# cristianpjensen/thesis-pai-reconstruction

Measured on NVIDIA B200. Metric: pix2pix_gan_train_images_per_sec_256x256, higher is better.
Workload: dtype bf16

## Files before the change

include/pai_b200.h:

```cpp
#ifndef PAI_B200_H
#define PAI_B200_H

#ifdef __cplusplus
extern "C" {
#endif

#define PAI_ACT_NONE 0
#define PAI_ACT_LEAKY 1
#define PAI_ACT_RELU 2
#define PAI_ACT_TANH 3

#define PAI_DTYPE_F32 0
#define PAI_DTYPE_BF16 1

const char* pai_last_error(void);
int pai_version(void);
int pai_reserve_sms(int n);

int pai_conv4x4_fprop(const void* x, int n, int h, int w, int cin, int x_ld, const void* w_packed, int cout,
                      int cout_pad, int stride, const float* bias, int act, float slope, void* y, int y_ld,
                      int y_f32, int n_tile, float* splitk_ws, void* stream);

int pai_conv4x4_fprop_dual(const void* x, int n, int h, int w, int cin, int x_ld, const void* w_packed, int cout,
                           int cout_pad, int stride, const float* bias, int act, float slope, void* y, int y_ld, void* y2,
                           int y2_ld, int act2, int n_tile, void* stream);

int pai_convT4x4s2_fprop(const void* x, int n, int h, int w, int cin, int x_ld, const void* w_packed, int cout,
                         int cout_pad, const float* bias, int act, float slope, void* y, int y_ld, int y_f32,
                         int n_tile, float* splitk_ws, void* stream);
int pai_conv4x4_fprop_bnstats(const void* x, int n, int h, int w, int cin, int x_ld, const void* w_packed, int cout,
                              int cout_pad, int stride, const float* bias, void* y, int y_ld, int n_tile,
                              float* bn_partials, int bn_rows, void* stream);
int pai_convT4x4s2_fprop_bnstats(const void* x, int n, int h, int w, int cin, int x_ld, const void* w_packed, int cout,
                                 int cout_pad, const float* bias, void* y, int y_ld, int n_tile, float* bn_partials,
                                 int bn_rows, void* stream);
int pai_conv4x4_dgrad_act(const void* gy, int n, int h, int w, int cout, int gy_ld, const void* w_packed_dgrad, int cin,
                          int cin_pad, const void* saved_act, float slope, void* gx, int gx_ld, int n_tile,
                          float* colsum_partials, int rows, void* stream);

int pai_conv4x4_wgrad(const void* x, int n, int h, int w, int cin, int x_ld, const void* gy, int cout, int gy_ld,
                      int stride, float* dw, int splitk, void* stream);
int pai_convT4x4s2_wgrad(const void* x, int n, int h, int w, int cin, int x_ld, const void* gy, int cout, int gy_ld,
                         float* dw, int splitk, void* stream);

int pai_ssim_psnr_fwd(const void* pred, const void* target, int dtype, int n, int h, int w, int denormalize,
                      float* ssim_sum, float* band_sum, float* sse, float* full_map, void* stream);
int pai_ssim_psnr_bwd(const void* pred, const void* target, int dtype, int n, int h, int w, int denormalize,
                      const float* g_ssim_sum, const float* g_sse, void* workspace, void* grad_pred, void* stream);
long long pai_ssim_bwd_workspace_bytes(int n, int h, int w);

int pai_bn_stats(const void* x, long long m, int c, int ld, float* sums, void* stream);
int pai_bn_finalize(const float* sums, long long m, int c, const float* gamma, const float* beta, float eps,
                    float momentum, int training, float* running_mean, float* running_var, float* scale_shift,
                    void* stream);
int pai_bn_finalize_partials(const float* sums, int nparts, long long m, int c, const float* gamma, const float* beta,
                             float eps, float momentum, int training, float* running_mean, float* running_var,
                             float* scale_shift, void* stream);
int pai_bn_apply_act(const void* x, long long m, int c, int ld, const float* scale_shift, void* out1, int ld1,
                     int act1, void* out2, int ld2, int act2, float slope, void* stream);
int pai_bn_bwd_reduce(const void* x, long long m, int c, int ld, const float* scale_shift, const void* g1, int ldg1,
                      int act1, const void* g2, int ldg2, int act2, float slope, float* sums, void* stream);
int pai_bn_bwd_apply(const void* x, long long m, int c, int ld, const float* scale_shift, const void* g1, int ldg1,
                     int act1, const void* g2, int ldg2, int act2, float slope, const float* sums,
                     const float* gamma, void* dx, int lddx, void* stream);
int pai_act_bwd(const void* x, long long m, int c, int ld, const void* g1, int ldg1, int act1, const void* g2, int ldg2,
                int act2, float slope, float* sums2c, void* dx, int lddx, void* stream);
int pai_colsum(const void* x, long long m, int c, int ld, float* sums2c, void* stream);
int pai_bn_small_ok(long long m, int c, int operands);
int pai_bn_small_fwd(const void* x, long long m, int c, int ld, const float* gamma, const float* beta, float eps,
                     float momentum, float* running_mean, float* running_var, float* scale_shift, void* out1, int ld1,
                     int act1, void* out2, int ld2, int act2, float slope, const float* mask, int pixels_per_image,
                     void* stream);
int pai_bn_small_bwd(const void* x, long long m, int c, int ld, const float* scale_shift, const void* g1, int ldg1,
                     int act1, const void* g2, int ldg2, int act2, float slope, const float* mask, int pixels_per_image,
                     const float* gamma, float* sums, void* dx, int lddx, void* stream);

int pai_smallc_conv_fprop(const float* plane0, const float* plane1, int cin, int n, int ih, int iw, int oh, int ow,
                          int stride, int flip, const float* w, const float* bias, int c, void* out1, int ld1,
                          int act1, void* out2, int ld2, int act2, float slope, void* stream);
int pai_smallc_conv_wgrad(const void* a, int lda, int c, const float* plane0, const float* plane1, int cin, int n,
                          int ih, int iw, int oh, int ow, int stride, int flip, float* dw, void* stream);

int pai_im2col4x4(const float* plane0, const float* plane1, int cin, int n, int ih, int iw, int oh, int ow, int stride,
                  int flip, void* col, void* stream);
int pai_pointwise_gemm(const void* x, long long m, int cin, int x_ld, const void* w_packed, int cout, int cout_pad,
                       const float* bias, int act, float slope, void* y, int y_ld, int y_f32, void* y2, int y2_ld,
                       int act2, int n_tile, int k_valid, void* stream);
int pai_pointwise_wgrad(const void* u, long long m, int cu, int u_ld, const void* s, int cs, int s_ld, float* dw,
                        int splitk, void* stream);
int pai_col2im4x4s2(const float* p, int ldp, int n, int h, int w, const float* bias, int act, float* out,
                    void* stream);

int pai_thin_conv4x4s2_fprop(const float* plane0, const float* plane1, int cin, int n, int ih, int iw,
                             const void* w_packed, int cout, const float* bias, void* out1, int ld1, int act1, void* out2,
                             int ld2, int act2, float slope, void* stream);
int pai_thin_conv4x4s2_wgrad(const void* u, int u_ld, int c, const float* plane0, const float* plane1, int cin, int n,
                             int ih, int iw, float* dw, void* stream);
int pai_thin_convT4x4s2_plane(const void* x, int n, int h, int w, int c, int x_ld, const void* w_taps, const float* bias,
                              int act, float* out, void* stream);
int pai_col2im4x4s1(const float* p, int ldp, int n, int h, int w, float* out, void* stream);

int pai_to_uint8(const float* x, long long count, unsigned char* out, void* stream);
int pai_afmhot_u8(const float* img, int n, long long hw, unsigned char* out, void* stream);

int pai_adam_pack_conv4x4(float* w, const float* grad, float* exp_avg, float* exp_avg_sq, int a, int b, float beta1,
                          float beta2, float step_size, float inv_bias_correction2_sqrt, float eps, void* pack1,
                          void* pack2, int b_pad, const float* dyn, void* stream);
int pai_adam_pack_conv4x4_multi(int count, float* const* ws, const float* const* grads, float* const* exp_avgs,
                                float* const* exp_avg_sqs, const int* as, const int* bs, void* const* pack1s,
                                void* const* pack2s, const int* b_pads, float beta1, float beta2, float step_size,
                                float inv_bias_correction2_sqrt, float eps, const float* dyn, void* stream);
int pai_adam_multi(int count, float* const* params, const float* const* grads, float* const* exp_avgs,
                   float* const* exp_avg_sqs, const int* numels, float beta1, float beta2, float step_size,
                   float inv_bias_correction2_sqrt, float eps, const float* dyn, void* stream);
int pai_adam_prepare(int* step, float lr, float beta1, float beta2, float* dyn, void* stream);
int pai_ema_multi(int count, float* const* shadows, const float* const* params, const int* numels, float one_minus_decay,
                  void* stream);
int pai_wgrad_finish(float* dw_tap_major, long long ab, float* grad, int zero_src, void* stream);

int pai_conv3x3_fprop(const void* x, int n, int h, int w, int cin, int x_ld, const void* w_packed, int cout,
                      int cout_pad, const float* bias, int act, float slope, void* y, int y_ld, int y_f32, int n_tile,
                      float* splitk_ws, void* stream);
int pai_conv3x3_wgrad(const void* x, int n, int h, int w, int cin, int x_ld, const void* gy, int cout, int gy_ld,
                      float* dw, void* stream);
int pai_maxpool2_fwd(const void* x, int n, int h, int w, int c, int ldx, void* y, int ldy, void* stream);
int pai_maxpool2_bwd(const void* x, int n, int h, int w, int c, int ldx, const void* gy, int ldgy, void* gx, int ldgx,
                     void* stream);
int pai_upsample2_fwd(const void* x, int n, int h, int w, int c, int ldx, void* y, int ldy, void* stream);
int pai_upsample2_bwd(const void* gy, int n, int h, int w, int c, int ldgy, void* gx, int ldgx, void* stream);
int pai_add_act(const void* a, int lda, const void* b, int ldb, long long m, int c, int act, float slope, void* out,
                int ldo, void* stream);
int pai_scale_rows_fwd(const void* x, int ldx, const float* s, long long m, int c, int act, void* out, int ldo,
                       void* stream);
int pai_scale_rows_bwd(const void* x, int ldx, const float* s, const void* g, int ldg, long long m, int c, int act,
                       void* gx, int ldgx, float* gs, void* stream);
int pai_scale_channels(const void* x, int ldx, const float* mask, int n, long long hw, int c, void* out, int ldo,
                       void* stream);
int pai_conv_plane_to_wide(const float* plane, int n, int h, int w, int k, int pad, int flip, const float* wt,
                           const float* bias, int c, int act, float slope, void* out, int ldo, void* stream);
int pai_conv_wide_to_plane(const void* x, int n, int h, int w, int c, int ldx, int k, int pad, const float* wt,
                           const float* bias, int act, float* out, void* stream);
int pai_conv_plane_wide_wgrad(const float* plane, const void* wide, int ldw, int n, int h, int w, int c, int k, int pad,
                              int flip, float* dw, void* stream);
int pai_gconv4_3x3_fprop(const void* x, int n, int h, int w, int c, int ldx, const float* wt, const float* bias, void* y,
                         int ldy, void* stream);
int pai_gconv4_3x3_wgrad(const void* x, int ldx, const void* gy, int ldg, int n, int h, int w, int c, float* dw,
                         void* stream);

// ... 47 lines not shown
```

thesis-pai-reconstruction_b200/csrc/elementwise.cu:

```cuda
#include "pai_common.cuh"
#include "pai_kernels.h"

namespace pai {

static constexpr int kEwThreads = 256;

struct Vec8 {
    float v[8];
};
__device__ __forceinline__ Vec8 load8(const __nv_bfloat16* p) {
    const uint4 u = *reinterpret_cast<const uint4*>(p);
    const __nv_bfloat162* h = reinterpret_cast<const __nv_bfloat162*>(&u);
    Vec8 r;
#pragma unroll
    for (int i = 0; i < 4; ++i) {
        const float2 f = __bfloat1622float2(h[i]);
        r.v[2 * i] = f.x;
        r.v[2 * i + 1] = f.y;
    }
    return r;
}
__device__ __forceinline__ uint4 load_raw(const __nv_bfloat16* p) { return *reinterpret_cast<const uint4*>(p); }
__device__ __forceinline__ Vec8 unpack8(const uint4& u) {
    const __nv_bfloat162* h = reinterpret_cast<const __nv_bfloat162*>(&u);
    Vec8 r;
#pragma unroll
    for (int i = 0; i < 4; ++i) {
        const float2 f = __bfloat1622float2(h[i]);
        r.v[2 * i] = f.x;
        r.v[2 * i + 1] = f.y;
    }
    return r;
}
__device__ __forceinline__ void store8(__nv_bfloat16* p, const Vec8& r) {
    uint4 u;
    __nv_bfloat162* h = reinterpret_cast<__nv_bfloat162*>(&u);
#pragma unroll
    for (int i = 0; i < 4; ++i) h[i] = __floats2bfloat162_rn(r.v[2 * i], r.v[2 * i + 1]);
    *reinterpret_cast<uint4*>(p) = u;
}
__device__ __forceinline__ Vec8 loadf8(const float* p) {
    Vec8 r;
    const float4 a = *reinterpret_cast<const float4*>(p), b = *reinterpret_cast<const float4*>(p + 4);
    r.v[0] = a.x, r.v[1] = a.y, r.v[2] = a.z, r.v[3] = a.w, r.v[4] = b.x, r.v[5] = b.y, r.v[6] = b.z, r.v[7] = b.w;
    return r;
}
__device__ __forceinline__ float act_fwd(float z, int act, float slope) {
    if (act == PAI_ACT_LEAKY) return z > 0.f ? z : z * slope;
    if (act == PAI_ACT_RELU) return fmaxf(z, 0.f);
    return z;
}
__device__ __forceinline__ float act_grad(float z, int act, float slope) {
    if (act == PAI_ACT_LEAKY) return z > 0.f ? 1.f : slope;
// ... 630 lines not shown

static const size_t kSmallSmemMax = 200 * 1024;

int pai_bn_small_ok(long long m, int c, int operands) {
    return m > 0 && c > 0 && c % 8 == 0 && operands >= 1 && operands <= 3 && (size_t)m * 16 * operands <= kSmallSmemMax;
}

int pai_bn_small_fwd(const void* x, long long m, int c, int ld, const float* gamma, const float* beta, float eps,
                     float momentum, float* running_mean, float* running_var, float* scale_shift, void* out1, int ld1,
                     int act1, void* out2, int ld2, int act2, float slope, const float* mask, int pixels_per_image,
                     void* stream) {
    PAI_REQUIRE(x && scale_shift && out1 && m > 0, "pai_bn_small_fwd: null pointer / empty input");
    PAI_REQUIRE(pai_bn_small_ok(m, c, 1), "pai_bn_small_fwd: m=%lld c=%d does not fit one block per 8 channels", m, c);
    PAI_REQUIRE(ew_ok(8, x, ld) && ew_ok(8, out1, ld1) && (out2 == nullptr || ew_ok(8, out2, ld2)),
                "pai_bn_small_fwd: bad stride / alignment (c=%d)", c);
    PAI_REQUIRE(act1 != PAI_ACT_TANH && act2 != PAI_ACT_TANH, "pai_bn_small_fwd: tanh is not a BatchNorm consumer");
    PAI_REQUIRE(mask == nullptr || pixels_per_image > 0, "pai_bn_small_fwd: mask needs pixels_per_image");
    static DeviceOnce once;
    const int dev = current_device();
    if (dev < 0) return -1;
    if (once.need(dev)) {
        PAI_CUDA_OK(cudaFuncSetAttribute(bn_small_fwd_kernel, cudaFuncAttributeMaxDynamicSharedMemorySize, (int)kSmallSmemMax));
        once.mark(dev);
    }
    PAI_CUDA_OK(launch_pdl(bn_small_fwd_kernel, dim3((unsigned)(c / 8)), dim3(kSmallThreads), (size_t)m * 16, (cudaStream_t)stream, 1,
                           (const bf16*)x, (int)m, c, ld, gamma, beta, eps, momentum, running_mean, running_var, scale_shift,
                           (bf16*)out1, ld1, act1, (bf16*)out2, ld2, act2, slope, mask, pixels_per_image > 0 ? pixels_per_image : 1));
    return 0;
}

int pai_bn_small_bwd(const void* x, long long m, int c, int ld, const float* scale_shift, const void* g1, int ldg1,
                     int act1, const void* g2, int ldg2, int act2, float slope, const float* mask, int pixels_per_image,
                     const float* gamma, float* sums, void* dx, int lddx, void* stream) {
    PAI_REQUIRE(x && scale_shift && g1 && sums && dx && m > 0, "pai_bn_small_bwd: null pointer / empty input");
    const int operands = g2 != nullptr ? 3 : 2;
    PAI_REQUIRE(pai_bn_small_ok(m, c, operands), "pai_bn_small_bwd: m=%lld c=%d does not fit one block per 8 channels", m, c);
    PAI_REQUIRE(ew_ok(8, x, ld) && ew_ok(8, g1, ldg1) && (g2 == nullptr || ew_ok(8, g2, ldg2)) && ew_ok(8, dx, lddx),
                "pai_bn_small_bwd: bad stride / alignment (c=%d)", c);
    PAI_REQUIRE(mask == nullptr || pixels_per_image > 0, "pai_bn_small_bwd: mask needs pixels_per_image");
    static DeviceOnce once;
    const int dev = current_device();
    if (dev < 0) return -1;
    if (once.need(dev)) {
        PAI_CUDA_OK(cudaFuncSetAttribute(bn_small_bwd_kernel, cudaFuncAttributeMaxDynamicSharedMemorySize, (int)kSmallSmemMax));
        once.mark(dev);
    }
    PAI_CUDA_OK(launch_pdl(bn_small_bwd_kernel, dim3((unsigned)(c / 8)), dim3(kSmallBwdThreads), (size_t)m * 16 * operands,
                           (cudaStream_t)stream, 1, (const bf16*)x, (int)m, c, ld, scale_shift, (const bf16*)g1, ldg1, act1,
                           (const bf16*)g2, ldg2, act2, slope, mask, pixels_per_image > 0 ? pixels_per_image : 1, gamma, sums,
                           (bf16*)dx, lddx));
    return 0;
}

int pai_colsum(const void* x, long long m, int c, int ld, float* sums2c, void* stream) {
    PAI_REQUIRE(x && sums2c && m > 0, "pai_colsum: null pointer / empty input");
    cudaStream_t st = (cudaStream_t)stream;
    if (!ew_ok(c, x, ld)) {
        PAI_REQUIRE(c > 0 && c % 8 == 0 && ld % 8 == 0 && (reinterpret_cast<uintptr_t>(x) & 15) == 0,
                    "pai_colsum: bad channel count / stride / alignment (c=%d)", c);
        PAI_CUDA_OK(cudaMemsetAsync(sums2c, 0, sizeof(float) * 2 * c, st));
        const int ry = (int)(m < 64 ? m : 64);
        colsum_wide_kernel<<<dim3((c / 8 + kEwThreads - 1) / kEwThreads, ry), kEwThreads, 0, st>>>((const bf16*)x, m, c, ld, sums2c);
        PAI_CUDA_OK(cudaGetLastError());
        return 0;
    }
    PAI_CUDA_OK(cudaMemsetAsync(sums2c, 0, sizeof(float) * 2 * c, st));
    colsum_kernel<<<wave_grid<colsum_kernel>(m, c), kEwThreads, 0, st>>>((const bf16*)x, m, c, ld, sums2c);
    PAI_CUDA_OK(cudaGetLastError());
    return 0;
}

}

namespace pai {
__device__ __forceinline__ unsigned char to_u8(float x) {
    return (unsigned char)((int)(x * 255.999f) & 0xff);
}
__global__ void __launch_bounds__(256) to_uint8_kernel(const float* __restrict__ x, long long count, unsigned char* __restrict__ out) {
    for (long long i = blockIdx.x * 256LL + threadIdx.x; i < count; i += (long long)gridDim.x * 256) out[i] = to_u8(x[i]);
}
__global__ void __launch_bounds__(256) afmhot_u8_kernel(const float* __restrict__ img, int n, long long hw, unsigned char* __restrict__ out) {
    const long long total = (long long)n * hw;
    for (long long i = blockIdx.x * 256LL + threadIdx.x; i < total; i += (long long)gridDim.x * 256) {
        const long long b = i / hw, pix = i - b * hw;
        int idx = (int)(img[i] * 256.f);
        idx = idx < 0 ? 0 : (idx > 255 ? 255 : idx);
        const float v = (float)idx / 255.f;
        unsigned char* o = out + b * 3 * hw + pix;
        o[0] = to_u8(fminf(fmaxf(2.f * v, 0.f), 1.f));
        o[hw] = to_u8(fminf(fmaxf(2.f * v - 0.5f, 0.f), 1.f));
        o[2 * hw] = to_u8(fminf(fmaxf(2.f * v - 1.f, 0.f), 1.f));
    }
}
}

extern "C" {
int pai_to_uint8(const float* x, long long count, unsigned char* out, void* stream) {
    PAI_REQUIRE(x && out && count >= 0, "pai_to_uint8: bad arguments");
    if (count == 0) return 0;
    long long blocks = (count + 255) / 256;
    if (blocks > 148 * 16) blocks = 148 * 16;
    pai::to_uint8_kernel<<<(int)blocks, 256, 0, (cudaStream_t)stream>>>(x, count, out);
    PAI_CUDA_OK(cudaGetLastError());
    return 0;
}
int pai_afmhot_u8(const float* img, int n, long long hw, unsigned char* out, void* stream) {
// ... 67 lines not shown
```

thesis-pai-reconstruction_b200/csrc/igemm.cu:

```cuda
#include <stdio.h>
#include <stdlib.h>

#include "pai_common.cuh"
#include "pai_epilogue.cuh"
#include "pai_kernels.h"

namespace pai {

#ifdef PAI_PROFILE_ROLES
#define ROLE_T0() const long long _t0 = clock64()
#define ROLE_ADD(var) var += clock64() - _t0
#else
#define ROLE_T0()
#define ROLE_ADD(var)
#endif

static constexpr int kThreads = 256;
static constexpr int kFpropThreads = 384;
static constexpr int kMaxStages = 8;

struct __align__(8) PipeSmem {
    uint64_t full[kMaxStages];
    uint64_t empty[kMaxStages];
    uint64_t acc_full[2];
    uint64_t acc_empty[2];
    uint64_t mask_full[8];
    uint32_t tmem_base;
};

template <bool PAIR, bool MASKED>
__global__ void __launch_bounds__(kFpropThreads, 1)
igemm_fprop_kernel(const __grid_constant__ CUtensorMap tm_a, const __grid_constant__ CUtensorMap tm_b,
                   const __grid_constant__ IgemmOutMaps om, const IgemmFpropParams p) {
    pdl_launch_dependents();
    extern __shared__ uint8_t smem_raw[];
    __shared__ PipeSmem ps;
    __shared__ __align__(1024) uint4 stage_buf[8][32 * 8];
    uint8_t* smem = reinterpret_cast<uint8_t*>((reinterpret_cast<uintptr_t>(smem_raw) + 1023) & ~uintptr_t(1023));

    const int warp = threadIdx.x >> 5, lane = threadIdx.x & 31;
    const int n_tile = p.n_tile;
    const bool fused = p.fused_phases != 0;
    const uint32_t rank = PAIR ? cluster_ctarank() : 0u;
    const int cta_n = PAIR ? n_tile / 2 : n_tile;
    const uint32_t a_bytes = 128 * 128;
    const uint32_t b_bytes = (uint32_t)cta_n * 128;
    const int ksub = p.ksub;
    const uint32_t sub_bytes = a_bytes + (fused ? 4 : 1) * b_bytes;
    const uint32_t stage_bytes = (uint32_t)ksub * sub_bytes;
    const int stages = p.stages;
    const int num_kb = (fused ? 9 : p.ntaps) * p.kc_per_tap;
    const int acc_n = fused ? 4 * n_tile : n_tile;
    const uint32_t acc_cols = tmem_cols_for(acc_n);
    const int total_tiles = p.n_tiles * p.m_tiles * p.phases * p.splitk;
    const int worker = PAIR ? (int)(blockIdx.x >> 1) : (int)blockIdx.x;
    const int workers = PAIR ? (int)(gridDim.x >> 1) : (int)gridDim.x;

    if (warp == 0 && lane == 0) {
        tma_prefetch_desc(&tm_a);
        tma_prefetch_desc(&tm_b);
    }
    if (warp == 1 && lane == 0) {
        for (int s = 0; s < stages; ++s) {
            mbar_init(&ps.full[s], 1);
            mbar_init(&ps.empty[s], 1);
        }
        for (int a = 0; a < 2; ++a) {
            mbar_init(&ps.acc_full[a], 1);
            mbar_init(&ps.acc_empty[a], PAIR ? 16 : 8);
        }
        if (MASKED)
            for (int w = 0; w < 8; ++w) mbar_init(&ps.mask_full[w], 1);
        mbar_fence_init();
    }
    if (warp == 2) {
        if (PAIR)
            tmem_alloc_pair(&ps.tmem_base, 2 * acc_cols);
        else
            tmem_alloc(&ps.tmem_base, 2 * acc_cols);
    }
    tc_fence_before();
    if (PAIR)
        cluster_sync_all();
    else
        __syncthreads();
    tc_fence_after();
    const uint32_t tmem_base = ps.tmem_base;
    pdl_wait();

    long long prof_wait = 0, prof_wait2 = 0, prof_total = 0, prof_fence = 0, prof_issue = 0, prof_commit = 0;
    (void)prof_wait, (void)prof_wait2, (void)prof_total, (void)prof_fence, (void)prof_issue, (void)prof_commit;
    const int pidx = warp == 0 ? 0 : (warp == 2 ? 1 : (warp == 3 ? 2 : -1));
    if (pidx >= 0) {
        if (elect_one()) {
            constexpr int P = 3;
            int g = 0, mine = pidx;
            int stage = pidx;
            uint32_t phase = 0;
            while (stage >= stages) stage -= stages, phase ^= 1;
            const int brow = PAIR ? (int)rank * cta_n : 0;
#ifdef PAI_PROFILE_ROLES
            const long long tstart = clock64();
#endif
            for (int t = worker; t < total_tiles; t += workers) {
                int ks, tt, nt, r, mt, phase_idx, tw, th, tn;
                p.fd_splitk.divmod(t, tt, ks);
                p.fd_n_tiles.divmod(tt, r, nt);
                p.fd_m_tiles.divmod(r, phase_idx, mt);
                if (PAIR) mt = 2 * mt + (int)rank;
                p.fd_tiles_w.divmod(mt, mt, tw);
                p.fd_tiles_h.divmod(mt, tn, th);
                const int w0 = tw * p.bw, h0 = th * p.bh, n0 = tn * p.bn;
                const int col0 = nt * n_tile;
                const int kb_begin = num_kb * ks / p.splitk, kb_end = num_kb * (ks + 1) / p.splitk;
                const int g_end = g + (kb_end - kb_begin) / ksub;
                int pw0 = 0, ph0 = 0, pn0 = 0, pphase = 0;
                const bool pf = p.prefetch_taps != 0 && t + workers < total_tiles;
                if (pf) {
                    int r2, m2, tw2, th2, tn2;
                    p.fd_n_tiles.divmod(p.fd_splitk.quot(t + workers), r2, tn2);
                    p.fd_m_tiles.divmod(r2, pphase, m2);
                    if (PAIR) m2 = 2 * m2 + (int)rank;
                    p.fd_tiles_w.divmod(m2, m2, tw2);
                    p.fd_tiles_h.divmod(m2, tn2, th2);
                    pw0 = tw2 * p.bw, ph0 = th2 * p.bh, pn0 = tn2 * p.bn;
// ... 140 lines not shown
                                mbar_wait_u32(full0 + 8 * stage, phase);
                                ROLE_ADD(prof_wait);
                            }
                            tc_fence_after();
                            const uint32_t a_lo = a_lo0 + stage * stage_units, b_lo = a_lo + a_units;
                            if (elect_one()) {
                                umma_kblock_lo<PAIR, 4>(tmem_d, a_lo, b_lo, idesc, kb != kb_begin);
                                if (ksub > 1) umma_kblock_lo<PAIR, 4>(tmem_d, a_lo + sub_units, b_lo + sub_units, idesc, 1u);
                                umma_commit_u32<PAIR>(empty0 + 8 * stage);
                            }
                            if (++stage == stages) {
                                stage = 0;
                                phase ^= 1;
                            }
                        }
                    } else {
                        for (int kb = kb_begin; kb < kb_end; ++kb) {
                            mbar_wait_u32(full0 + 8 * stage, phase);
                            tc_fence_after();
                            const uint32_t a_lo = a_lo0 + stage * stage_units, b_lo = a_lo + a_units;
                            if (elect_one()) {
                                const uint32_t acc = kb != kb_begin;
                                if (kmma == 1)
                                    umma_kblock_lo<PAIR, 1>(tmem_d, a_lo, b_lo, idesc, acc);
                                else if (kmma == 2)
                                    umma_kblock_lo<PAIR, 2>(tmem_d, a_lo, b_lo, idesc, acc);
                                else
                                    umma_kblock_lo<PAIR, 3>(tmem_d, a_lo, b_lo, idesc, acc);
                                umma_commit_u32<PAIR>(empty0 + 8 * stage);
                            }
                            if (++stage == stages) {
                                stage = 0;
                                phase ^= 1;
                            }
                        }
                    }
                }
                if (elect_one()) umma_commit_u32<PAIR>(acc_full0 + 8 * a);
            }
#ifdef PAI_PROFILE_ROLES
            if (blockIdx.x == 0 && elect_one())
                printf("[roles] mma: total %lld cyc, waiting for full stages %lld, for a drained accumulator %lld, tiles %d, k-blocks/tile %d; unfused: fence %lld issue %lld commit %lld\n",
                       clock64() - tstart, prof_wait, prof_wait2, it, num_kb / p.splitk, prof_fence, prof_issue, prof_commit);
#endif
        }
    } else if (warp >= 4) {
        const int q = warp & 3;
        const int half = (warp - 4) >> 2;
        const int r = q * 32 + lane;
        const int rpos = (r % p.bw) | (((r / p.bw) % p.bh) << 8) | ((r / (p.bw * p.bh)) << 16);
        const int n_out = p.out2 != nullptr ? 2 : 1;
        const int qpos = __shfl_sync(0xffffffffu, rpos, 0);
        uint4* tile = stage_buf[warp - 4];
        uint32_t mask_phase = 0;
        const bool st_persist = fused || acc_n <= 128;
        float st_sum[8], st_sq[8];
#pragma unroll
        for (int j = 0; j < 8; ++j) st_sum[j] = st_sq[j] = 0.f;
        int st_col = -1;
        auto reduce_add = [&](float (&su)[8], float (&sq)[8], int col) {
#pragma unroll
            for (int j = 0; j < 8; ++j) {
                su[j] += __shfl_xor_sync(0xffffffffu, su[j], 8);
                su[j] += __shfl_xor_sync(0xffffffffu, su[j], 16);
                sq[j] += __shfl_xor_sync(0xffffffffu, sq[j], 8);
                sq[j] += __shfl_xor_sync(0xffffffffu, sq[j], 16);
            }
            if (lane < 8) {
                float* bp = p.bn_part + (size_t)blockIdx.x * (2 * p.cout) + col + lane * 8;
#pragma unroll
                for (int j = 0; j < 8; ++j) {
                    atomicAdd(bp + j, su[j]);
                    atomicAdd(bp + p.cout + j, sq[j]);
                }
            }
        };
        auto flush_stats = [&]() {
            if (st_col < 0) return;
            reduce_add(st_sum, st_sq, st_col);
#pragma unroll
            for (int j = 0; j < 8; ++j) st_sum[j] = st_sq[j] = 0.f;
            st_col = -1;
        };
        int it = 0;
        for (int t = worker; t < total_tiles; t += workers, ++it) {
            int nt, rr, mt, phase_idx, tw, th, tn;
            const int tt = p.fd_splitk.quot(t);
            p.fd_n_tiles.divmod(tt, rr, nt);
            p.fd_m_tiles.divmod(rr, phase_idx, mt);
            if (PAIR) mt = 2 * mt + (int)rank;
            p.fd_tiles_w.divmod(mt, mt, tw);
            p.fd_tiles_h.divmod(mt, tn, th);
            const int col0 = nt * n_tile;
            const int gw = tw * p.bw + (rpos & 255), gh = th * p.bh + ((rpos >> 8) & 255), gn = tn * p.bn + (rpos >> 16);
            const bool row_ok = (gw < p.gw) && (gh < p.gh) && (gn < p.gn);
            const int a = it & 1;
            const uint32_t acc_phase = (it >> 1) & 1;
            const bool fast = p.tma_out && (n_tile & 63) == 0 && col0 + n_tile <= p.cout &&
                              (p.bias == nullptr || (reinterpret_cast<uintptr_t>(p.bias) & 15) == 0);
            const int bw0 = tw * p.bw + (qpos & 255), bh0 = th * p.bh + ((qpos >> 8) & 255), bn0 = tn * p.bn + (qpos >> 16);
            const bool masked = MASKED && p.mask_src != nullptr && fast;
            auto mask_load = [&](int c) {
                __syncwarp();
                if (lane == 0) {
                    bulk_wait_group_read0();
                    mbar_expect_tx(&ps.mask_full[warp - 4], 32 * 128);
                    tma_load_4d(tile, &om.aux[fused ? c >> 6 : phase_idx], &ps.mask_full[warp - 4], col0 + (fused ? 0 : c),
                                bw0, bh0, bn0);
                }
            };
            if (masked && 64 * half < acc_n) mask_load(64 * half);
            {
                ROLE_T0();
                mbar_wait(&ps.acc_full[a], acc_phase);
                ROLE_ADD(prof_wait);
            }
#ifdef PAI_PROFILE_ROLES
            const long long twork = clock64();
#endif
            tc_fence_after();
            const uint32_t tmem_d = tmem_base + a * acc_cols + ((uint32_t)(q * 32) << 16);
            bool released = false;
            auto release_acc = [&]() {
                tc_fence_before();
                __syncwarp();
                if (lane == 0) {
                    if (PAIR)
                        mbar_arrive_leader_relaxed(&ps.acc_empty[a]);
                    else
                        mbar_arrive_relaxed(&ps.acc_empty[a]);
                }
                released = true;
            };
            if (fast) {
                const uint32_t rows_ok = __ballot_sync(0xffffffffu, row_ok);
                int item = 0;
                const int n_items = (acc_n >> 6) * n_out;
                const int last_item = ((n_items - 1) & 1) == half ? n_items - 1 : n_items - 2;
                for (int c = 0; c < acc_n; c += 64) {
                    const int oc = fused ? 0 : c;
                    for (int which = 0; which < n_out; ++which, ++item) {
                        if ((item & 1) != half) continue;
                        uint32_t v[64];
#pragma unroll
                        for (int j = 0; j < 4; ++j)
                            tmem_ld_16(tmem_d + (uint32_t)(c + 16 * j), *reinterpret_cast<uint32_t(*)[16]>(&v[16 * j]));
                        tmem_ld_wait();
                        if (item == last_item) release_acc();
                        const int act = which == 0 ? p.act : p.act2;
                        const float* bias_c = p.bias != nullptr ? p.bias + col0 + oc : nullptr;
                        if (masked) {
                            mbar_wait(&ps.mask_full[warp - 4], mask_phase);
                            mask_phase ^= 1;
                            mask_pack(v, p.mask_slope, tile, lane);
                        } else {
                            if (lane == 0) bulk_wait_group_read0();
                            __syncwarp();
                            if (act == PAI_ACT_LEAKY)
                                bias_act_pack<PAI_ACT_LEAKY>(v, bias_c, p.slope, tile, lane);
                            else if (act == PAI_ACT_RELU)
                                bias_act_pack<PAI_ACT_RELU>(v, bias_c, p.slope, tile, lane);
                            else if (act == PAI_ACT_TANH)
                                bias_act_pack<PAI_ACT_TANH>(v, bias_c, p.slope, tile, lane);
                            else
                                bias_act_pack<PAI_ACT_NONE>(v, bias_c, p.slope, tile, lane);
                        }
                        fence_proxy_async_smem();
                        __syncwarp();
                        if (lane == 0) {
                            tma_store_4d(which == 0 ? &om.out[fused ? c >> 6 : phase_idx] : &om.aux[0], tile, col0 + oc,
                                         bw0, bh0, bn0);
                            bulk_commit_group();
                        }
                        const bool stats = p.bn_part != nullptr && which == 0;
                        if (stats) {
                            if (st_persist && st_col != col0 + oc) {
                                flush_stats();
                                st_col = col0 + oc;
                            }
                            float cs[8], cq[8];
#pragma unroll
                            for (int j = 0; j < 8; ++j) cs[j] = cq[j] = 0.f;
#pragma unroll
                            for (int i = 0; i < 8; ++i) {
                                const int row = i * 4 + (lane >> 3), ch = lane & 7;
                                if ((rows_ok >> row) & 1u) {
                                    const uint4 val = tile[row * 8 + (ch ^ (row & 7))];
                                    const __nv_bfloat162* hv = reinterpret_cast<const __nv_bfloat162*>(&val);
#pragma unroll
                                    for (int j = 0; j < 4; ++j) {
                                        const float2 f = __bfloat1622float2(hv[j]);
                                        cs[2 * j] += f.x;
                                        cs[2 * j + 1] += f.y;
                                        cq[2 * j] = fmaf(f.x, f.x, cq[2 * j]);
                                        cq[2 * j + 1] = fmaf(f.y, f.y, cq[2 * j + 1]);
                                    }
                                }
                            }
                            if (st_persist) {
#pragma unroll
                                for (int j = 0; j < 8; ++j) st_sum[j] += cs[j], st_sq[j] += cq[j];
                            } else {
                                reduce_add(cs, cq, col0 + oc);
                            }
                        }
                        if (masked && c + 128 < acc_n) mask_load(c + 128);
                    }
                }
            } else {
                const long long off = p.out_phase_off[phase_idx] + (long long)gn * p.out_sn + (long long)gh * p.out_sh +
                                      (long long)gw * p.out_sw + col0;
                const long long off2 = (long long)gn * p.out2_sn + (long long)gh * p.out2_sh + (long long)gw * p.out2_sw + col0;
                const bool vec_ok = ((p.cout & 7) == 0) && ((off & 7) == 0) && ((off2 & 7) == 0);
                int step = 0;
                for (int cc = 0; cc < n_tile; cc += 16, ++step) {
                    if ((step & 1) != half) continue;
                    uint32_t v[16];
                    __syncwarp();
                    tmem_ld_16(tmem_d + (uint32_t)cc, v);
                    tmem_ld_wait();
                    if (!row_ok || col0 + cc >= p.cout) continue;
                    float f[16];
#pragma unroll
                    for (int j = 0; j < 16; ++j) {
                        float x = __uint_as_float(v[j]);
                        if (p.bias != nullptr && col0 + cc + j < p.cout) x += __ldg(p.bias + col0 + cc + j);
                        f[j] = x;
                    }
                    if (p.accumulate) {
                        float* o = reinterpret_cast<float*>(p.out) + off + cc;
                        if (col0 + cc + 16 <= p.cout && ((off + cc) & 3) == 0) {
#pragma unroll
                            for (int j = 0; j < 16; j += 4) red_add_v4(o + j, f[j], f[j + 1], f[j + 2], f[j + 3]);
                        } else {
#pragma unroll
                            for (int j = 0; j < 16; ++j)
                                if (col0 + cc + j < p.cout) atomicAdd(o + j, f[j]);
                        }
                    } else if (p.out_f32) {
                        float* o = reinterpret_cast<float*>(p.out) + off + cc;
                        if (col0 + cc + 16 <= p.cout && ((off + cc) & 3) == 0 && p.act == PAI_ACT_NONE) {
#pragma unroll
                            for (int j = 0; j < 16; j += 4)
                                *reinterpret_cast<float4*>(o + j) = make_float4(f[j], f[j + 1], f[j + 2], f[j + 3]);
                        } else {
#pragma unroll
                            for (int j = 0; j < 16; ++j)
                                if (col0 + cc + j < p.cout) o[j] = apply_act(f[j], p.act, p.slope);
                        }
                    } else {
                        store_bf16_16(reinterpret_cast<__nv_bfloat16*>(p.out) + off + cc, f, p.act, p.slope,
                                      vec_ok && col0 + cc + 16 <= p.cout, p.cout - (col0 + cc));
                    }
                    if (p.out2 != nullptr)
                        store_bf16_16(reinterpret_cast<__nv_bfloat16*>(p.out2) + off2 + cc, f, p.act2, p.slope,
                                      vec_ok && col0 + cc + 16 <= p.cout, p.cout - (col0 + cc));
                }
            }
            if (!released) release_acc();
// ... 191 lines not shown
    return ((m_tiles + 1) / 2) * n_tiles * phases >= 74;
}

int launch_igemm_fprop(const CUtensorMap& tm_a, const CUtensorMap& tm_b, const IgemmOutMaps& om, IgemmFpropParams p,
                       int m_tiles, int n_tiles, int phases, cudaStream_t stream) {
    const bool pair = p.pair != 0;
    const size_t sub_bytes = 128 * 128 + (size_t)(p.fused_phases ? 4 : 1) * (pair ? p.n_tile / 2 : p.n_tile) * 128;
    if (p.kmma <= 0 || p.kmma > 4) p.kmma = 4;
    if (p.splitk < 1) p.splitk = 1;
    {
        static const char* env = getenv("PAI_IGEMM_KSUB");
        const int num_kb = (p.fused_phases ? 9 : p.ntaps) * p.kc_per_tap;
        const bool even = p.fused_phases ? p.kc_per_tap % 2 == 0 : num_kb % (2 * p.splitk) == 0;
        p.ksub = (even && p.kmma == 4 && 3 * 2 * sub_bytes <= 192 * 1024 && !(env && env[0] == '1')) ? 2 : 1;
    }
    const size_t stage_bytes = sub_bytes * p.ksub;
    p.stages = pick_stages(stage_bytes, 192 * 1024);
    p.prefetch_taps = 0;
    if (getenv("PAI_L2_PREFETCH") != nullptr && p.splitk == 1) {
        if (p.fused_phases) {
            p.prefetch_taps = 1u;
        } else {
            for (int t = 0; t < p.ntaps && t < 32; ++t) {
                bool first = true;
                for (int u = 0; u < t; ++u) first = first && !(p.tap_c[u] == p.tap_c[t] && p.tap_p[u] == p.tap_p[t]);
                if (first) p.prefetch_taps |= 1u << t;
            }
        }
    }
    p.m_tiles = pair ? (m_tiles + 1) / 2 : m_tiles, p.n_tiles = n_tiles, p.phases = phases;
    const size_t smem = stage_bytes * p.stages + 1024;
    static DeviceOnce once;
    const int dev = current_device(), num_sms = persistent_ctas(dev);
    if (num_sms < 0) return -1;
    if (once.need(dev)) {
        PAI_CUDA_OK(cudaFuncSetAttribute(igemm_fprop_kernel<false, false>, cudaFuncAttributeMaxDynamicSharedMemorySize, 194 * 1024));
        PAI_CUDA_OK(cudaFuncSetAttribute(igemm_fprop_kernel<true, false>, cudaFuncAttributeMaxDynamicSharedMemorySize, 194 * 1024));
        PAI_CUDA_OK(cudaFuncSetAttribute(igemm_fprop_kernel<false, true>, cudaFuncAttributeMaxDynamicSharedMemorySize, 194 * 1024));
        PAI_CUDA_OK(cudaFuncSetAttribute(igemm_fprop_kernel<true, true>, cudaFuncAttributeMaxDynamicSharedMemorySize, 194 * 1024));
        once.mark(dev);
    }
    if (p.splitk < 1) p.splitk = 1;
    PAI_REQUIRE(!pair || (p.splitk == 1 && p.n_tile % 32 == 0), "igemm fprop: the CTA-pair kernel needs n_tile %% 32 == 0 and no split-K");
    p.fd_splitk = make_fastdiv(p.splitk), p.fd_n_tiles = make_fastdiv(n_tiles), p.fd_m_tiles = make_fastdiv(p.m_tiles);
    p.fd_tiles_w = make_fastdiv(p.tiles_w), p.fd_tiles_h = make_fastdiv(p.tiles_h), p.fd_kc = make_fastdiv(p.kc_per_tap);
    const long long total = (long long)p.m_tiles * n_tiles * phases * p.splitk;
    int grid;
    if (pair) {
        const long long pairs = total < num_sms / 2 ? total : num_sms / 2;
        grid = (int)(2 * pairs);
    } else {
        grid = (int)(total < num_sms ? total : num_sms);
    }
    if (p.mask_src != nullptr)
        PAI_REQUIRE(!p.out_f32 && p.splitk == 1 && !p.accumulate && (p.n_tile & 63) == 0 && p.cout % p.n_tile == 0 &&
                        (p.cout & 7) == 0 && p.bias == nullptr && p.act == PAI_ACT_NONE && p.out2 == nullptr &&
                        (reinterpret_cast<uintptr_t>(p.mask_src) & 15) == 0 && p.tma_out,
                    "igemm fprop: the fused activation backward needs a plain bf16 output with 16 B aligned rows, "
                    "cout %% 64 == 0 and no split-K (cout=%d n_tile=%d splitk=%d)", p.cout, p.n_tile, p.splitk);
    if (p.bn_part != nullptr) {
        PAI_REQUIRE(!p.out_f32 && p.splitk == 1 && !p.accumulate && (p.n_tile & 63) == 0 && p.cout % p.n_tile == 0 &&
                        (p.cout & 7) == 0 && p.bn_rows >= grid,
                    "igemm fprop: fused BatchNorm statistics need a bf16 output with cout %% 64 == 0, no split-K and "
                    "%d partial rows (cout=%d n_tile=%d splitk=%d rows=%d)", grid, p.cout, p.n_tile, p.splitk, p.bn_rows);
    }
    const int cl = pair ? 2 : 1;
    const dim3 g((unsigned)grid), b(kFpropThreads);
    if (pair && p.mask_src != nullptr)
        PAI_CUDA_OK(launch_pdl(igemm_fprop_kernel<true, true>, g, b, smem, stream, cl, tm_a, tm_b, om, p));
    else if (pair)
        PAI_CUDA_OK(launch_pdl(igemm_fprop_kernel<true, false>, g, b, smem, stream, cl, tm_a, tm_b, om, p));
    else if (p.mask_src != nullptr)
        PAI_CUDA_OK(launch_pdl(igemm_fprop_kernel<false, true>, g, b, smem, stream, cl, tm_a, tm_b, om, p));
    else
        PAI_CUDA_OK(launch_pdl(igemm_fprop_kernel<false, false>, g, b, smem, stream, cl, tm_a, tm_b, om, p));
    PAI_CUDA_OK(cudaGetLastError());
    return 0;
}

__global__ void __launch_bounds__(256)
splitk_finish_kernel(const float* __restrict__ ws, long long total, int cout, const float* __restrict__ bias, int act,
                     float slope, void* __restrict__ y, int y_ld, int y_f32) {
    pdl_launch_dependents();
    pdl_wait();
    for (long long i = (long long)blockIdx.x * blockDim.x + threadIdx.x; i < total; i += (long long)gridDim.x * blockDim.x) {
        const long long pix = i / cout;
        const int c = (int)(i - pix * cout);
        float v = ws[i];
        if (bias != nullptr) v += bias[c];
        v = apply_act(v, act, slope);
        if (y_f32)
            reinterpret_cast<float*>(y)[pix * y_ld + c] = v;
        else
            reinterpret_cast<__nv_bfloat16*>(y)[pix * y_ld + c] = __float2bfloat16_rn(v);
    }
}

int launch_splitk_finish(const float* ws, long long pixels, int cout, const float* bias, int act, float slope, void* y,
                         int y_ld, int y_f32, cudaStream_t stream) {
    const long long total = pixels * cout;
    long long blocks = (total + 255) / 256;
    const int sms = sm_count(current_device());
    if (sms < 0) return -1;
    if (blocks > sms * 8) blocks = sms * 8;
    PAI_CUDA_OK(launch_pdl(splitk_finish_kernel, dim3((unsigned)blocks), dim3(256), 0, stream, 1, ws, total, cout, bias, act, slope, y, y_ld, y_f32));
    PAI_CUDA_OK(cudaGetLastError());
    return 0;
}

int launch_igemm_wgrad(const CUtensorMap& tm_u, const CUtensorMap& tm_s, IgemmWgradParams p, cudaStream_t stream) {
    const size_t stage_bytes = (size_t)(2 * p.mb + p.nbt) * 8192;
    p.stages = pick_stages(stage_bytes, 196 * 1024);
    const size_t smem = stage_bytes * p.stages + 1024;
    static DeviceOnce once;
    const int dev = current_device(), num_sms = persistent_ctas(dev);
    if (num_sms < 0) return -1;
    if (once.need(dev)) {
        PAI_CUDA_OK(cudaFuncSetAttribute(igemm_wgrad_kernel, cudaFuncAttributeMaxDynamicSharedMemorySize, 200 * 1024));
        once.mark(dev);
    }
    const long long units = (long long)p.tiles * p.kblocks;
    long long grid = units / 4 > p.tiles ? units / 4 : p.tiles;
    if (grid > num_sms) grid = num_sms;
    if (grid < 1) grid = 1;
    if (p.max_ctas > 0 && grid > p.max_ctas) grid = p.max_ctas;
// ... 7 lines not shown
```

thesis-pai-reconstruction_b200/csrc/pai_api.cu:

```cuda
#include <stdarg.h>
#include <stdio.h>
#include <stdlib.h>
#include <string.h>

#include <cudaTypedefs.h>

#include "pai_common.cuh"
#include "pai_kernels.h"

namespace pai {

static thread_local char g_err[512] = "";

void set_error(const char* fmt, ...) {
    va_list ap;
    va_start(ap, fmt);
    vsnprintf(g_err, sizeof(g_err), fmt, ap);
    va_end(ap);
}

int cuda_fail(cudaError_t e, const char* what) {
    set_error("CUDA error %d (%s) at %s", (int)e, cudaGetErrorString(e), what);
    return -1;
}
// ... 83 lines not shown
    PixBox b;
    b.bw = pow2_ge(gw) < m ? pow2_ge(gw) : m;
    int rest = m / b.bw;
    b.bh = pow2_ge(gh) < rest ? pow2_ge(gh) : rest;
    b.bn = rest / b.bh;
    b.tiles_w = (gw + b.bw - 1) / b.bw;
    b.tiles_h = (gh + b.bh - 1) / b.bh;
    b.tiles_n = (gn + b.bn - 1) / b.bn;
    return b;
}

static int map_unit(CUtensorMap* m, const void* base, int n, int h, int w, int c, int ld, const PixBox& b) {
    uint64_t dims[5] = {(uint64_t)c, (uint64_t)w, 1, (uint64_t)h, (uint64_t)n};
    uint64_t str[4] = {(uint64_t)ld * 2, (uint64_t)w * ld * 2, (uint64_t)w * ld * 2, (uint64_t)h * w * ld * 2};
    uint32_t box[5] = {64, (uint32_t)b.bw, 1, (uint32_t)b.bh, (uint32_t)b.bn};
    return encode_tmap_bf16(m, base, 5, dims, str, box);
}
static int map_split(CUtensorMap* m, const void* base, int n, int h, int w, int c, const PixBox& b) {
    uint64_t dims[5] = {(uint64_t)2 * c, (uint64_t)w / 2, 2, (uint64_t)h / 2, (uint64_t)n};
    uint64_t str[4] = {(uint64_t)2 * c * 2, (uint64_t)w * c * 2, (uint64_t)2 * w * c * 2, (uint64_t)h * w * c * 2};
    uint32_t box[5] = {64, (uint32_t)b.bw, 1, (uint32_t)b.bh, (uint32_t)b.bn};
    return encode_tmap_bf16(m, base, 5, dims, str, box);
}
static void s2_tap(int k, int* q, int* par) {
    static const int Q[4] = {-1, 0, 0, 1}, P[4] = {1, 0, 1, 0};
    *q = Q[k];
    *par = P[k];
}
static const int kTd[2][2] = {{0, -1}, {1, 0}};

static bool aligned16(const void* p) { return (reinterpret_cast<uintptr_t>(p) & 15) == 0; }

static int map_out(CUtensorMap* m, const void* base, int cout, int gw, int gh, int gn, long long sw, long long sh,
                   long long sn, const PixBox& b) {
    const int bw = b.bw < 32 ? b.bw : 32, bh = b.bh < 32 / bw ? b.bh : 32 / bw, bn = 32 / (bw * bh);
    if (sh == 0) sh = (long long)gw * sw;
    uint64_t dims[4] = {(uint64_t)cout, (uint64_t)gw, (uint64_t)gh, (uint64_t)gn};
    uint64_t str[3] = {(uint64_t)sw * 2, (uint64_t)sh * 2, (uint64_t)sn * 2};
    uint32_t box[4] = {64, (uint32_t)bw, (uint32_t)bh, (uint32_t)bn};
    return encode_tmap_bf16(m, base, 4, dims, str, box);
}

static int map_outputs(IgemmOutMaps* om, IgemmFpropParams& p, int nmaps, const PixBox& b) {
    p.tma_out = 0;
    const bool ok = !p.out_f32 && !p.accumulate && (p.cout & 7) == 0 && aligned16(p.out) && p.out_sw % 8 == 0 &&
                    p.out_sh % 8 == 0 && p.out_sn % 8 == 0 &&
                    (p.out2 == nullptr || (aligned16(p.out2) && p.out2_sw % 8 == 0 && p.out2_sh % 8 == 0 && p.out2_sn % 8 == 0));
    if (!ok) return 0;
    for (int j = 0; j < nmaps; ++j) {
        PAI_REQUIRE(p.out_phase_off[j] % 8 == 0, "igemm fprop: phase offset %lld is not 16 B aligned", p.out_phase_off[j]);
        int rc = map_out(&om->out[j], static_cast<const __nv_bfloat16*>(p.out) + p.out_phase_off[j], p.cout, p.gw, p.gh,
                         p.gn, p.out_sw, p.out_sh, p.out_sn, b);
        if (rc) return rc;
        if (p.mask_src != nullptr) {
            rc = map_out(&om->aux[j], static_cast<const __nv_bfloat16*>(p.mask_src) + p.out_phase_off[j], p.cout, p.gw,
                         p.gh, p.gn, p.out_sw, p.out_sh, p.out_sn, b);
            if (rc) return rc;
        }
    }
    if (p.out2 != nullptr) {
        int rc = map_out(&om->aux[0], p.out2, p.cout, p.gw, p.gh, p.gn, p.out2_sw, p.out2_sh, p.out2_sn, b);
        if (rc) return rc;
    }
    p.tma_out = 1;
    return 0;
}

static int auto_n_tile(int cout_pad, long long m_tiles_x_phases) {
    static const int cand[5] = {256, 128, 64, 32, 16};
    int best = 0;
    for (int i = 0; i < 5; ++i) {
        if (cout_pad % cand[i]) continue;
        if (best == 0) best = cand[i];
        if (m_tiles_x_phases * (cout_pad / cand[i]) >= 148) return cand[i];
        best = cand[i] >= 128 ? cand[i] : best;
        if (cand[i] <= 128) break;
    }
    return best;
}

static int pick_splitk(const void* ws, long long tiles, int num_kb) {
    if (ws == nullptr || tiles > 74 || num_kb < 8) return 1;
    long long s = 148 / tiles;
    if (s > num_kb / 2) s = num_kb / 2;
    return s < 2 ? 1 : (int)s;
}

}

using namespace pai;

extern "C" {

const char* pai_last_error(void) { return g_err; }
int pai_version(void) { return 100; }

int pai_reserve_sms(int n) {
    PAI_REQUIRE(n >= 0 && n <= 64, "pai_reserve_sms: reservation must be in 0..64 (got %d)", n);
    __atomic_store_n(&g_reserved_sms, n, __ATOMIC_RELAXED);
    return 0;
}

static int conv4x4_fprop_impl(const void* x, int n, int h, int w, int cin, int x_ld, const void* w_packed, int cout,
                              int cout_pad, int stride, const float* bias, int act, float slope, void* y, int y_ld,
                              int y_f32, int n_tile, float* splitk_ws, float* bn_part, int bn_rows, void* stream,
                              void* y2 = nullptr, int y2_ld = 0, int act2 = PAI_ACT_NONE) {
    PAI_REQUIRE(x && w_packed && y, "pai_conv4x4_fprop: null pointer");
    PAI_REQUIRE(stride == 1 || stride == 2, "pai_conv4x4_fprop: stride must be 1 or 2 (got %d)", stride);
    PAI_REQUIRE(cin > 0 && cin % 64 == 0, "pai_conv4x4_fprop: cin must be a multiple of 64 (got %d)", cin);
    PAI_REQUIRE(cout_pad % 16 == 0 && cout <= cout_pad, "pai_conv4x4_fprop: bad cout %d / cout_pad %d", cout, cout_pad);
    PAI_REQUIRE(aligned16(x) && aligned16(w_packed) && x_ld % 8 == 0, "pai_conv4x4_fprop: x / w must be 16 B aligned");
    int ho, wo;
    if (stride == 2) {
        PAI_REQUIRE(h % 2 == 0 && w % 2 == 0 && x_ld == cin, "pai_conv4x4_fprop: stride 2 needs even h,w and dense x");
        ho = h / 2;
        wo = w / 2;
    } else {
        PAI_REQUIRE(h >= 2 && w >= 2, "pai_conv4x4_fprop: stride 1 needs h,w >= 2");
        ho = h - 1;
        wo = w - 1;
    }
    PixBox b = pick_box(wo, ho, n, 128);
    if (n_tile <= 0) n_tile = auto_n_tile(cout_pad, (long long)b.tiles_w * b.tiles_h * b.tiles_n);
    PAI_REQUIRE(n_tile >= 16 && n_tile <= 256 && n_tile % 16 == 0 && cout_pad % n_tile == 0,
                "pai_conv4x4_fprop: bad n_tile %d for cout_pad %d", n_tile, cout_pad);
    CUtensorMap tm_a, tm_b;
    int rc = stride == 2 ? map_split(&tm_a, x, n, h, w, cin, b) : map_unit(&tm_a, x, n, h, w, cin, x_ld, b);
    if (rc) return rc;
    const int m_tiles = b.tiles_w * b.tiles_h * b.tiles_n;
    const int splitk = pick_splitk(splitk_ws, (long long)m_tiles * (cout_pad / n_tile), 16 * (cin / 64));
    const bool pair = igemm_fprop_use_pair(n_tile, m_tiles, cout_pad / n_tile, 1, splitk);
    uint64_t bd[2] = {(uint64_t)16 * cin, (uint64_t)cout_pad};
    uint64_t bs[1] = {(uint64_t)16 * cin * 2};
    uint32_t bb[2] = {64, (uint32_t)(pair ? n_tile / 2 : n_tile)};
    rc = encode_tmap_bf16(&tm_b, w_packed, 2, bd, bs, bb);
    if (rc) return rc;

    IgemmFpropParams p;
    memset(&p, 0, sizeof(p));
    IgemmOutMaps om;
    memset(&om, 0, sizeof(om));
    p.pair = pair;
    p.bw = b.bw, p.bh = b.bh, p.bn = b.bn, p.tiles_w = b.tiles_w, p.tiles_h = b.tiles_h;
    p.gw = wo, p.gh = ho, p.gn = n;
    p.n_tile = n_tile, p.cout = cout, p.kc_per_tap = cin / 64, p.ntaps = 16;
    for (int ky = 0; ky < 4; ++ky)
        for (int kx = 0; kx < 4; ++kx) {
            int t = ky * 4 + kx;
            if (stride == 2) {
                int qx, px, qy, py;
                s2_tap(kx, &qx, &px);
                s2_tap(ky, &qy, &py);
                p.tap_c[t] = px * cin, p.tap_w[t] = qx, p.tap_p[t] = py, p.tap_h[t] = qy;
            } else {
                p.tap_c[t] = 0, p.tap_w[t] = kx - 1, p.tap_p[t] = 0, p.tap_h[t] = ky - 1;
            }
        }
    p.b_rows_per_phase = cout_pad;
    p.bn_part = bn_part, p.bn_rows = bn_rows;
    p.splitk = splitk;
    if (p.splitk > 1) {
        p.out_sn = (long long)ho * wo * cout, p.out_sh = (long long)wo * cout, p.out_sw = cout;
        p.out_f32 = 1, p.accumulate = 1, p.out = splitk_ws;
        int rc2 = launch_igemm_fprop(tm_a, tm_b, om, p, m_tiles, cout_pad / n_tile, 1, (cudaStream_t)stream);
        if (rc2) return rc2;
        return launch_splitk_finish(splitk_ws, (long long)n * ho * wo, cout, bias, act, slope, y, y_ld, y_f32,
                                    (cudaStream_t)stream);
    }
    p.out_sn = (long long)ho * wo * y_ld, p.out_sh = (long long)wo * y_ld, p.out_sw = y_ld;
    p.bias = bias, p.act = act, p.slope = slope, p.out_f32 = y_f32, p.out = y;
    if (y2 != nullptr) {
        PAI_REQUIRE(!y_f32 && y2_ld % 8 == 0 && aligned16(y2) && aligned16(y) && y_ld % 8 == 0 && cout % 64 == 0,
                    "pai_conv4x4_fprop_dual: two bf16 outputs need cout %% 64 == 0 and 16 B aligned rows");
        p.out2 = y2, p.act2 = act2;
        p.out2_sn = (long long)ho * wo * y2_ld, p.out2_sh = (long long)wo * y2_ld, p.out2_sw = y2_ld;
    }
    rc = map_outputs(&om, p, 1, b);
    if (rc) return rc;
    return launch_igemm_fprop(tm_a, tm_b, om, p, m_tiles, cout_pad / n_tile, 1, (cudaStream_t)stream);
}

int pai_conv4x4_fprop_dual(const void* x, int n, int h, int w, int cin, int x_ld, const void* w_packed, int cout,
                           int cout_pad, int stride, const float* bias, int act, float slope, void* y, int y_ld, void* y2,
                           int y2_ld, int act2, int n_tile, void* stream) {
    PAI_REQUIRE(y2 != nullptr, "pai_conv4x4_fprop_dual: null second output");
    return conv4x4_fprop_impl(x, n, h, w, cin, x_ld, w_packed, cout, cout_pad, stride, bias, act, slope, y, y_ld, 0, n_tile,
                              nullptr, nullptr, 0, stream, y2, y2_ld, act2);
}

int pai_conv4x4_fprop(const void* x, int n, int h, int w, int cin, int x_ld, const void* w_packed, int cout,
                      int cout_pad, int stride, const float* bias, int act, float slope, void* y, int y_ld,
                      int y_f32, int n_tile, float* splitk_ws, void* stream) {
    return conv4x4_fprop_impl(x, n, h, w, cin, x_ld, w_packed, cout, cout_pad, stride, bias, act, slope, y, y_ld, y_f32,
                              n_tile, splitk_ws, nullptr, 0, stream);
}
int pai_conv4x4_fprop_bnstats(const void* x, int n, int h, int w, int cin, int x_ld, const void* w_packed, int cout,
                              int cout_pad, int stride, const float* bias, void* y, int y_ld, int n_tile,
                              float* bn_partials, int bn_rows, void* stream) {
    PAI_REQUIRE(bn_partials != nullptr && bn_rows > 0, "pai_conv4x4_fprop_bnstats: null partial-sum buffer");
    return conv4x4_fprop_impl(x, n, h, w, cin, x_ld, w_packed, cout, cout_pad, stride, bias, PAI_ACT_NONE, 0.f, y, y_ld, 0,
                              n_tile, nullptr, bn_partials, bn_rows, stream);
}

static int convT4x4s2_fprop_impl(const void* x, int n, int h, int w, int cin, int x_ld, const void* w_packed, int cout,
                                 int cout_pad, const float* bias, int act, float slope, void* y, int y_ld, int y_f32,
                                 int n_tile, float* splitk_ws, float* bn_part, int bn_rows, void* stream,
                                 const void* mask_src = nullptr, float mask_slope = 0.f) {
    PAI_REQUIRE(x && w_packed && y, "pai_convT4x4s2_fprop: null pointer");
    PAI_REQUIRE(cin > 0 && cin % 64 == 0, "pai_convT4x4s2_fprop: cin must be a multiple of 64 (got %d)", cin);
    PAI_REQUIRE(cout_pad % 16 == 0 && cout <= cout_pad, "pai_convT4x4s2_fprop: bad cout %d / cout_pad %d", cout, cout_pad);
    PAI_REQUIRE(aligned16(x) && aligned16(w_packed) && x_ld % 8 == 0 && x_ld >= cin,
                "pai_convT4x4s2_fprop: x / w must be 16 B aligned");
    PixBox b = pick_box(w, h, n, 128);
    if (n_tile <= 0) n_tile = auto_n_tile(cout_pad, 4LL * b.tiles_w * b.tiles_h * b.tiles_n);
    PAI_REQUIRE(n_tile >= 16 && n_tile <= 256 && n_tile % 16 == 0 && cout_pad % n_tile == 0,
                "pai_convT4x4s2_fprop: bad n_tile %d for cout_pad %d", n_tile, cout_pad);
    CUtensorMap tm_a, tm_b;
    int rc = map_unit(&tm_a, x, n, h, w, cin, x_ld, b);
    if (rc) return rc;
    const int m_tiles = b.tiles_w * b.tiles_h * b.tiles_n;
    const int splitk = pick_splitk(splitk_ws, 4LL * m_tiles * (cout_pad / n_tile), 4 * (cin / 64));
    const bool fuse = splitk == 1 && cout == 64 && cout_pad == 64 && n_tile == 64 && !y_f32 && y_ld % 8 == 0 &&
                      aligned16(y) && (bias == nullptr || aligned16(bias)) && getenv("PAI_NO_PHASE_FUSION") == nullptr;
    const bool pair = fuse ? igemm_fprop_use_pair(n_tile, m_tiles, 1, 1, 1)
                           : igemm_fprop_use_pair(n_tile, m_tiles, cout_pad / n_tile, 4, splitk);
    uint64_t bd[2] = {(uint64_t)4 * cin, (uint64_t)4 * cout_pad};
    uint64_t bs[1] = {(uint64_t)4 * cin * 2};
    uint32_t bb[2] = {64, (uint32_t)(pair ? n_tile / 2 : n_tile)};
    rc = encode_tmap_bf16(&tm_b, w_packed, 2, bd, bs, bb);
    if (rc) return rc;

    IgemmFpropParams p;
    memset(&p, 0, sizeof(p));
    IgemmOutMaps om;
    memset(&om, 0, sizeof(om));
    p.pair = pair;
    p.bw = b.bw, p.bh = b.bh, p.bn = b.bn, p.tiles_w = b.tiles_w, p.tiles_h = b.tiles_h;
    p.gw = w, p.gh = h, p.gn = n;
    p.n_tile = n_tile, p.cout = cout, p.kc_per_tap = cin / 64, p.ntaps = 4;
    for (int py = 0; py < 2; ++py)
        for (int px = 0; px < 2; ++px)
            for (int ty = 0; ty < 2; ++ty)
                for (int tx = 0; tx < 2; ++tx) {
                    int i = (py * 2 + px) * 4 + ty * 2 + tx;
                    p.tap_c[i] = 0, p.tap_w[i] = kTd[px][tx], p.tap_p[i] = 0, p.tap_h[i] = kTd[py][ty];
                }
    p.b_rows_per_phase = cout_pad;
    p.bn_part = bn_part, p.bn_rows = bn_rows;
    p.mask_src = mask_src, p.mask_slope = mask_slope;
    const long long wo = 2LL * w;
    p.splitk = splitk;
    const long long ld = p.splitk > 1 ? cout : y_ld;
    p.out_sn = 4LL * h * w * ld, p.out_sh = 2 * wo * ld, p.out_sw = 2LL * ld;
    for (int py = 0; py < 2; ++py)
        for (int px = 0; px < 2; ++px) p.out_phase_off[py * 2 + px] = (py * wo + px) * ld;
    if (fuse) {
        p.fused_phases = 1;
        static const int col_of_phase[4] = {0, 1, 3, 2};
        static const int box_order[9] = {4, 0, 1, 2, 3, 5, 6, 7, 8};
        const bool merge_ok = getenv("PAI_NO_PHASE_MERGE") == nullptr;
        for (int bi = 0; bi < 9; ++bi) {
            const int bx = box_order[bi];
            const int dy = bx / 3 - 1, dx = bx % 3 - 1;
            p.box_h[bi] = dy, p.box_w[bi] = dx;
            int nu = 0;
            for (int col = 0; col < 4; ++col)
                for (int ph = 0; ph < 4; ++ph) {
                    if (col_of_phase[ph] != col) continue;
                    const int py = ph >> 1, px = ph & 1;
                    for (int ty = 0; ty < 2; ++ty)
                        for (int tx = 0; tx < 2; ++tx)
                            if (kTd[py][ty] == dy && kTd[px][tx] == dx) {
                                p.box_users[bi][nu] = ph * 4 + ty * 2 + tx;
                                p.box_col[bi][nu] = col;
                                ++nu;
                            }
                }
            p.box_nu[bi] = nu;
            bool consecutive = nu > 1;
            for (int u = 1; u < nu; ++u) consecutive = consecutive && p.box_col[bi][u] == p.box_col[bi][u - 1] + 1;
            p.box_merge[bi] = merge_ok && consecutive;
            for (; nu < 4; ++nu) p.box_users[bi][nu] = -1, p.box_col[bi][nu] = 0;
        }
        for (int py = 0; py < 2; ++py)
            for (int px = 0; px < 2; ++px) p.out_phase_off[col_of_phase[py * 2 + px]] = (py * wo + px) * ld;
        p.bias = bias, p.act = act, p.slope = slope, p.out_f32 = 0, p.out = y;
        rc = map_outputs(&om, p, 4, b);
        if (rc) return rc;
        return launch_igemm_fprop(tm_a, tm_b, om, p, m_tiles, 1, 1, (cudaStream_t)stream);
    }
    if (p.splitk > 1) {
        p.out_f32 = 1, p.accumulate = 1, p.out = splitk_ws;
        int rc2 = launch_igemm_fprop(tm_a, tm_b, om, p, m_tiles, cout_pad / n_tile, 4, (cudaStream_t)stream);
        if (rc2) return rc2;
        return launch_splitk_finish(splitk_ws, 4LL * n * h * w, cout, bias, act, slope, y, y_ld, y_f32,
                                    (cudaStream_t)stream);
    }
    p.bias = bias, p.act = act, p.slope = slope, p.out_f32 = y_f32, p.out = y;
    rc = map_outputs(&om, p, 4, b);
    if (rc) return rc;
    return launch_igemm_fprop(tm_a, tm_b, om, p, m_tiles, cout_pad / n_tile, 4, (cudaStream_t)stream);
}

int pai_convT4x4s2_fprop(const void* x, int n, int h, int w, int cin, int x_ld, const void* w_packed, int cout,
                         int cout_pad, const float* bias, int act, float slope, void* y, int y_ld, int y_f32,
                         int n_tile, float* splitk_ws, void* stream) {
    return convT4x4s2_fprop_impl(x, n, h, w, cin, x_ld, w_packed, cout, cout_pad, bias, act, slope, y, y_ld, y_f32, n_tile,
                                 splitk_ws, nullptr, 0, stream);
}
int pai_convT4x4s2_fprop_bnstats(const void* x, int n, int h, int w, int cin, int x_ld, const void* w_packed, int cout,
                                 int cout_pad, const float* bias, void* y, int y_ld, int n_tile, float* bn_partials,
                                 int bn_rows, void* stream) {
    PAI_REQUIRE(bn_partials != nullptr && bn_rows > 0, "pai_convT4x4s2_fprop_bnstats: null partial-sum buffer");
    return convT4x4s2_fprop_impl(x, n, h, w, cin, x_ld, w_packed, cout, cout_pad, bias, PAI_ACT_NONE, 0.f, y, y_ld, 0,
                                 n_tile, nullptr, bn_partials, bn_rows, stream);
}

int pai_conv4x4_dgrad_act(const void* gy, int n, int h, int w, int cout, int gy_ld, const void* w_packed_dgrad, int cin,
                          int cin_pad, const void* saved_act, float slope, void* gx, int gx_ld, int n_tile,
                          float* colsum_partials, int rows, void* stream) {
    PAI_REQUIRE(saved_act != nullptr, "pai_conv4x4_dgrad_act: null saved activation");
    PAI_REQUIRE(colsum_partials == nullptr || rows > 0, "pai_conv4x4_dgrad_act: bad partial-sum buffer");
    return convT4x4s2_fprop_impl(gy, n, h, w, cout, gy_ld, w_packed_dgrad, cin, cin_pad, nullptr, PAI_ACT_NONE, 0.f, gx,
                                 gx_ld, 0, n_tile, nullptr, colsum_partials, rows, stream, saved_act, slope);
}

static int wgrad_common(const void* u, int un, int uh, int uw, int cu, int u_ld, const void* s, int sh, int sw,
                        int cs, int s_ld, int stride, float* dw, int splitk, cudaStream_t stream, const char* who) {
    PAI_REQUIRE(u && s && dw, "%s: null pointer", who);
    PAI_REQUIRE(cu % 64 == 0 && cs % 64 == 0, "%s: channel counts (%d rows, %d cols) must be multiples of 64", who, cu,
                cs);
    PAI_REQUIRE(aligned16(u) && aligned16(s) && u_ld % 8 == 0 && s_ld % 8 == 0, "%s: operands must be 16 B aligned",
                who);
    PixBox b = pick_box(uw, uh, un, 64);
    CUtensorMap tm_u, tm_s;
    int rc = map_unit(&tm_u, u, un, uh, uw, cu, u_ld, b);
    if (rc) return rc;
    if (stride == 2) {
        PAI_REQUIRE(s_ld == cs && sh % 2 == 0 && sw % 2 == 0, "%s: the stride-2 operand must be dense with even h,w",
                    who);
        rc = map_split(&tm_s, s, un, sh, sw, cs, b);
    } else {
        rc = map_unit(&tm_s, s, un, sh, sw, cs, s_ld, b);
    }
    if (rc) return rc;
    IgemmWgradParams p;
    memset(&p, 0, sizeof(p));
    p.bw = b.bw, p.bh = b.bh, p.bn = b.bn, p.tiles_w = b.tiles_w, p.tiles_h = b.tiles_h, p.tiles_n = b.tiles_n;
    p.cu = cu, p.cs = cs, p.out = dw;
    for (int ky = 0; ky < 4; ++ky)
        for (int kx = 0; kx < 4; ++kx) {
            int t = ky * 4 + kx;
            if (stride == 2) {
                int qx, px, qy, py;
                s2_tap(kx, &qx, &px);
                s2_tap(ky, &qy, &py);
                p.tap_c[t] = px * cs, p.tap_w[t] = qx, p.tap_p[t] = py, p.tap_h[t] = qy;
            } else if (stride == 1) {
                p.tap_c[t] = 0, p.tap_w[t] = kx - 1, p.tap_p[t] = 0, p.tap_h[t] = ky - 1;
            }
        }
    if (stride == 3)
        for (int t = 0; t < 9; ++t) p.tap_c[t] = 0, p.tap_w[t] = t % 3 - 1, p.tap_p[t] = 0, p.tap_h[t] = t / 3 - 1;
    const int ntaps = stride == 0 ? 1 : (stride == 3 ? 9 : 16);
    p.kblocks = b.tiles_w * b.tiles_h * b.tiles_n;
    p.cs_blocks = cs / 64;
    const int nb_total = ntaps * p.cs_blocks;
    p.nbt = nb_total % 4 == 0 ? 4 : (nb_total % 2 == 0 ? 2 : 1);
    p.n_groups = nb_total / p.nbt;
    p.mb = cu > 128 ? 2 : 1;
    p.tiles = ((cu + 128 * p.mb - 1) / (128 * p.mb)) * p.n_groups;
    p.max_ctas = splitk > 0 ? splitk * p.tiles : 0;
    return launch_igemm_wgrad(tm_u, tm_s, p, stream);
}

int pai_conv4x4_wgrad(const void* x, int n, int h, int w, int cin, int x_ld, const void* gy, int cout, int gy_ld,
                      int stride, float* dw, int splitk, void* stream) {
// ... 113 lines not shown
```

thesis-pai-reconstruction_b200/csrc/pai_common.cuh:

```cuda
#pragma once
#include <cuda.h>
#include <cuda_bf16.h>
#include <cuda_runtime.h>
#include <stdint.h>
#include <stdio.h>

namespace pai {

void set_error(const char* fmt, ...);
int cuda_fail(cudaError_t e, const char* what);
#define PAI_CUDA_OK(expr)                                                   \
    do {                                                                    \
        cudaError_t _e = (expr);                                            \
        if (_e != cudaSuccess) return ::pai::cuda_fail(_e, #expr);          \
    } while (0)
#define PAI_REQUIRE(cond, ...)                                              \
    do {                                                                    \
        if (!(cond)) {                                                      \
            ::pai::set_error(__VA_ARGS__);                                  \
            return -2;                                                      \
        }                                                                   \
    } while (0)

struct DeviceOnce {
// ... 51 lines not shown

__device__ __forceinline__ void mbar_init(uint64_t* bar, uint32_t count) {
    asm volatile("mbarrier.init.shared::cta.b64 [%0], %1;" ::"r"(smem_u32(bar)), "r"(count) : "memory");
}
__device__ __forceinline__ void mbar_fence_init() {
    asm volatile("fence.mbarrier_init.release.cluster;" ::: "memory");
}
__device__ __forceinline__ void mbar_expect_tx(uint64_t* bar, uint32_t bytes) {
    asm volatile("mbarrier.arrive.expect_tx.shared::cta.b64 _, [%0], %1;" ::"r"(smem_u32(bar)), "r"(bytes)
                 : "memory");
}
__device__ __forceinline__ void mbar_arrive(uint64_t* bar) {
    asm volatile("mbarrier.arrive.shared::cta.b64 _, [%0];" ::"r"(smem_u32(bar)) : "memory");
}
__device__ __forceinline__ bool mbar_try_wait(uint64_t* bar, uint32_t parity) {
    uint32_t ok;
    asm volatile(
        "{\n"
        ".reg .pred p;\n"
        "mbarrier.try_wait.parity.shared::cta.b64 p, [%1], %2;\n"
        "selp.u32 %0, 1, 0, p;\n"
        "}\n"
        : "=r"(ok)
        : "r"(smem_u32(bar)), "r"(parity)
        : "memory");
    return ok != 0;
}
__device__ __forceinline__ void mbar_wait(uint64_t* bar, uint32_t parity) {
    if (mbar_try_wait(bar, parity)) return;
    long long t0 = clock64();
    while (!mbar_try_wait(bar, parity)) {
        if (clock64() - t0 > 4000000000LL) {
            printf("pai: mbarrier wait timed out (block %d,%d,%d thread %d)\n", blockIdx.x, blockIdx.y,
                   blockIdx.z, threadIdx.x);
            __trap();
        }
    }
}

__device__ __forceinline__ void tma_load_2d(void* dst, const CUtensorMap* map, uint64_t* bar, int c0, int c1) {
    asm volatile(
        "cp.async.bulk.tensor.2d.shared::cluster.global.mbarrier::complete_tx::bytes [%0], [%1, {%3, %4}], [%2];"
        ::"r"(smem_u32(dst)), "l"(reinterpret_cast<uint64_t>(map)), "r"(smem_u32(bar)), "r"(c0), "r"(c1)
        : "memory");
}
__device__ __forceinline__ void tma_load_5d(void* dst, const CUtensorMap* map, uint64_t* bar, int c0, int c1,
                                            int c2, int c3, int c4) {
    asm volatile(
        "cp.async.bulk.tensor.5d.shared::cluster.global.mbarrier::complete_tx::bytes [%0], [%1, {%3, %4, %5, %6, "
        "%7}], [%2];" ::"r"(smem_u32(dst)),
        "l"(reinterpret_cast<uint64_t>(map)), "r"(smem_u32(bar)), "r"(c0), "r"(c1), "r"(c2), "r"(c3), "r"(c4)
        : "memory");
}
__device__ __forceinline__ void tma_prefetch_5d(const CUtensorMap* map, int c0, int c1, int c2, int c3, int c4) {
    asm volatile("cp.async.bulk.prefetch.tensor.5d.L2.global.tile [%0, {%1, %2, %3, %4, %5}];" ::"l"(
                     reinterpret_cast<uint64_t>(map)),
                 "r"(c0), "r"(c1), "r"(c2), "r"(c3), "r"(c4)
                 : "memory");
}
__device__ __forceinline__ void tma_load_4d(void* dst, const CUtensorMap* map, uint64_t* bar, int c0, int c1, int c2,
                                            int c3) {
    asm volatile(
        "cp.async.bulk.tensor.4d.shared::cluster.global.mbarrier::complete_tx::bytes [%0], [%1, {%3, %4, %5, %6}], [%2];"
        ::"r"(smem_u32(dst)), "l"(reinterpret_cast<uint64_t>(map)), "r"(smem_u32(bar)), "r"(c0), "r"(c1), "r"(c2), "r"(c3)
        : "memory");
}
__device__ __forceinline__ void tma_store_4d(const CUtensorMap* map, const void* src, int c0, int c1, int c2, int c3) {
    asm volatile("cp.async.bulk.tensor.4d.global.shared::cta.bulk_group [%0, {%2, %3, %4, %5}], [%1];" ::"l"(
                     reinterpret_cast<uint64_t>(map)),
                 "r"(smem_u32(src)), "r"(c0), "r"(c1), "r"(c2), "r"(c3)
                 : "memory");
}
__device__ __forceinline__ void bulk_commit_group() { asm volatile("cp.async.bulk.commit_group;" ::: "memory"); }
__device__ __forceinline__ void bulk_wait_group_read0() { asm volatile("cp.async.bulk.wait_group.read 0;" ::: "memory"); }
__device__ __forceinline__ void bulk_wait_group0() { asm volatile("cp.async.bulk.wait_group 0;" ::: "memory"); }
__device__ __forceinline__ void tma_prefetch_desc(const CUtensorMap* map) {
    asm volatile("prefetch.tensormap [%0];" ::"l"(reinterpret_cast<uint64_t>(map)) : "memory");
}

__device__ __forceinline__ void tmem_alloc(uint32_t* dst_smem, uint32_t ncols) {
    asm volatile("tcgen05.alloc.cta_group::1.sync.aligned.shared::cta.b32 [%0], %1;" ::"r"(smem_u32(dst_smem)),
                 "r"(ncols)
                 : "memory");
    asm volatile("tcgen05.relinquish_alloc_permit.cta_group::1.sync.aligned;" ::: "memory");
}
__device__ __forceinline__ void tmem_dealloc(uint32_t taddr, uint32_t ncols) {
    asm volatile("tcgen05.dealloc.cta_group::1.sync.aligned.b32 %0, %1;" ::"r"(taddr), "r"(ncols) : "memory");
}
__device__ __forceinline__ void tc_fence_before() { asm volatile("tcgen05.fence::before_thread_sync;" ::: "memory"); }
__device__ __forceinline__ void tc_fence_after() { asm volatile("tcgen05.fence::after_thread_sync;" ::: "memory"); }

__device__ __forceinline__ void umma_bf16_ss(uint32_t tmem_d, uint64_t desc_a, uint64_t desc_b, uint32_t idesc,
                                             uint32_t accumulate) {
    asm volatile(
        "{\n"
        ".reg .pred p;\n"
        "setp.ne.b32 p, %4, 0;\n"
        "tcgen05.mma.cta_group::1.kind::f16 [%0], %1, %2, %3, p;\n"
        "}\n" ::"r"(tmem_d),
        "l"(desc_a), "l"(desc_b), "r"(idesc), "r"(accumulate)
        : "memory");
}
__device__ __forceinline__ void umma_bf16_acc(uint32_t tmem_d, uint64_t desc_a, uint64_t desc_b, uint32_t idesc) {
    asm volatile(
        "{\n"
        ".reg .pred p;\n"
// ... 185 lines not shown
```

thesis-pai-reconstruction_b200/csrc/pai_epilogue.cuh:

```cuda
#pragma once
#include "pai_common.cuh"
#include "pai_kernels.h"

namespace pai {

__device__ __forceinline__ uint32_t tmem_cols_for(int n) {
    uint32_t c = 32;
    while ((int)c < n) c <<= 1;
    return c;
}

__device__ __forceinline__ float apply_act(float v, int act, float slope) {
    if (act == PAI_ACT_LEAKY) return v > 0.f ? v : v * slope;
    if (act == PAI_ACT_RELU) return fmaxf(v, 0.f);
    if (act == PAI_ACT_TANH) return tanhf(v);
    return v;
}

__device__ __forceinline__ void red_add_v4(float* addr, float a, float b, float c, float d) {
    asm volatile("red.global.add.v4.f32 [%0], {%1, %2, %3, %4};" ::"l"(addr), "f"(a), "f"(b), "f"(c), "f"(d)
                 : "memory");
}

__device__ __forceinline__ void store_bf16_16(__nv_bfloat16* o, const float (&f)[16], int act, float slope, bool vec,
                                              int valid) {
    if (vec) {
        uint32_t w[8];
#pragma unroll
        for (int j = 0; j < 8; ++j) {
            __nv_bfloat162 h = __floats2bfloat162_rn(apply_act(f[2 * j], act, slope), apply_act(f[2 * j + 1], act, slope));
            w[j] = *reinterpret_cast<uint32_t*>(&h);
        }
        reinterpret_cast<uint4*>(o)[0] = make_uint4(w[0], w[1], w[2], w[3]);
        reinterpret_cast<uint4*>(o)[1] = make_uint4(w[4], w[5], w[6], w[7]);
    } else {
#pragma unroll
        for (int j = 0; j < 16; ++j)
            if (j < valid) o[j] = __float2bfloat16_rn(apply_act(f[j], act, slope));
    }
}

template <int ACT>
__device__ __forceinline__ float act_t(float v, float slope) {
    if (ACT == PAI_ACT_LEAKY) return fmaxf(v, v * slope);
    if (ACT == PAI_ACT_RELU) return fmaxf(v, 0.f);
    if (ACT == PAI_ACT_TANH) return tanhf(v);
    return v;
}
template <int ACT>
__device__ __forceinline__ void bias_act_pack(const uint32_t (&v)[64], const float* __restrict__ bias, float slope,
                                              uint4* tile, int lane) {
#pragma unroll
    for (int ch = 0; ch < 8; ++ch) {
        float f[8];
#pragma unroll
        for (int k = 0; k < 8; ++k) f[k] = __uint_as_float(v[8 * ch + k]);
        if (bias != nullptr) {
            const float4 b0 = __ldg(reinterpret_cast<const float4*>(bias + 8 * ch));
            const float4 b1 = __ldg(reinterpret_cast<const float4*>(bias + 8 * ch) + 1);
            f[0] += b0.x, f[1] += b0.y, f[2] += b0.z, f[3] += b0.w;
            f[4] += b1.x, f[5] += b1.y, f[6] += b1.z, f[7] += b1.w;
        }
        uint32_t w[4];
#pragma unroll
        for (int k = 0; k < 4; ++k) {
            __nv_bfloat162 h = __floats2bfloat162_rn(act_t<ACT>(f[2 * k], slope), act_t<ACT>(f[2 * k + 1], slope));
            w[k] = *reinterpret_cast<uint32_t*>(&h);
        }
        tile[lane * 8 + (ch ^ (lane & 7))] = make_uint4(w[0], w[1], w[2], w[3]);
    }
}

__device__ __forceinline__ void mask_pack(const uint32_t (&v)[64], float slope, uint4* tile, int lane) {
#pragma unroll
    for (int ch = 0; ch < 8; ++ch) {
        const uint4 m = tile[lane * 8 + (ch ^ (lane & 7))];
        const __nv_bfloat162* mh = reinterpret_cast<const __nv_bfloat162*>(&m);
        uint32_t w[4];
#pragma unroll
        for (int k = 0; k < 4; ++k) {
            const float2 mf = __bfloat1622float2(mh[k]);
            const float a = __uint_as_float(v[8 * ch + 2 * k]) * (mf.x > 0.f ? 1.f : slope);
            const float b = __uint_as_float(v[8 * ch + 2 * k + 1]) * (mf.y > 0.f ? 1.f : slope);
            __nv_bfloat162 h = __floats2bfloat162_rn(a, b);
            w[k] = *reinterpret_cast<uint32_t*>(&h);
        }
        tile[lane * 8 + (ch ^ (lane & 7))] = make_uint4(w[0], w[1], w[2], w[3]);
    }
}


__device__ __forceinline__ uint32_t sw128_off(int r, int c) { return (uint32_t)r * 128u + (uint32_t)((c ^ (r & 7)) << 4); }

__device__ __forceinline__ void fence_proxy_async_smem() { asm volatile("fence.proxy.async.shared::cta;" ::: "memory"); }

}
```

thesis-pai-reconstruction_b200/csrc/pai_kernels.h:

```cpp
#pragma once
#include <cuda.h>
#include <cuda_runtime.h>
#include <stdint.h>

#include "../../include/pai_b200.h"

namespace pai {

struct FastDiv {
    uint32_t mul, shift, div;
#ifdef __CUDACC__
    __device__ __forceinline__ int quot(int n) const { return (int)((__umulhi((uint32_t)n, mul) + (uint32_t)n) >> shift); }
    __device__ __forceinline__ void divmod(int n, int& q, int& r) const {
        q = quot(n);
        r = n - q * (int)div;
    }
#endif
};
inline FastDiv make_fastdiv(int d) {
    FastDiv f;
    f.div = (uint32_t)d;
    uint32_t s = 0;
    while ((1u << s) < (uint32_t)d) ++s;
    f.shift = s;
    f.mul = (uint32_t)(((1ull << 32) * ((1ull << s) - (uint64_t)d)) / (uint64_t)d + 1);
    return f;
}

struct IgemmFpropParams {
    int bw, bh, bn;
    int tiles_w, tiles_h;
    int gw, gh, gn;
    int n_tile;
    int cout;
    int kc_per_tap, ntaps;
    int stages;
    int ksub;
    unsigned prefetch_taps;
    int m_tiles, n_tiles, phases;
    int tap_c[16], tap_w[16], tap_p[16], tap_h[16];
    int b_rows_per_phase;
    long long out_sn, out_sh, out_sw;
    long long out_phase_off[4];
    const float* bias;
    int act;
    float slope;
    int out_f32;
    void* out;
    void* out2;
    int act2;
    long long out2_sn, out2_sh, out2_sw;
    FastDiv fd_splitk, fd_n_tiles, fd_m_tiles, fd_tiles_w, fd_tiles_h, fd_kc;
    int fused_phases;
    int box_w[9], box_h[9];
    int box_users[9][4];
    int box_nu[9], box_col[9][4], box_merge[9];
    int kmma;
    float* bn_part;
    int bn_rows;
    const void* mask_src;
    float mask_slope;
    int pair;
    int splitk;
    int accumulate;
    int tma_out;
};

struct IgemmOutMaps {
    CUtensorMap out[4];
    CUtensorMap aux[4];
};

struct IgemmWgradParams {
    int bw, bh, bn;
    int tiles_w, tiles_h, tiles_n;
    int kblocks;
    int mb;
    int nbt;
    int cs_blocks;
    int n_groups;
    int tiles;
    int max_ctas;
    int cu, cs;
    int stages;
    int tap_c[16], tap_w[16], tap_p[16], tap_h[16];
    float* out;
};

bool igemm_fprop_use_pair(int n_tile, long long m_tiles, int n_tiles, int phases, int splitk);
int launch_igemm_fprop(const CUtensorMap& tm_a, const CUtensorMap& tm_b, const IgemmOutMaps& om, IgemmFpropParams p,
                       int m_tiles, int n_tiles, int phases, cudaStream_t stream);
int launch_splitk_finish(const float* ws, long long pixels, int cout, const float* bias, int act, float slope, void* y,
                         int y_ld, int y_f32, cudaStream_t stream);
int launch_igemm_wgrad(const CUtensorMap& tm_u, const CUtensorMap& tm_s, IgemmWgradParams p, cudaStream_t stream);

}
```

thesis-pai-reconstruction_b200/csrc/thin.cu:

```cuda
#include <stdlib.h>

#include "pai_common.cuh"
#include "pai_epilogue.cuh"
#include "pai_kernels.h"

namespace pai {

#ifdef PAI_PROFILE_ROLES
#define TROLE_T0() const long long _t0 = clock64()
#define TROLE_ADD(var) var += clock64() - _t0
#else
#define TROLE_T0()
#define TROLE_ADD(var)
#endif

static constexpr int kThinFpropThreads = 16 * 32;

struct ThinFpropParams {
    const float* p0;
    const float* p1;
    int n, ih, iw, oh, ow;
    const __nv_bfloat16* w;
    int cout;
    const float* bias;
    __nv_bfloat16* out1;
    int ld1, act1;
    __nv_bfloat16* out2;
    int ld2, act2;
    float slope;
    long long total_pix;
    int tiles;
    FastDiv fd_ow, fd_oh;
};

struct __align__(8) ThinPipe {
    uint64_t a_full[2], a_empty[2], acc_full[2], acc_empty[2];
    uint32_t tmem_base;
};

template <int ACT>
__device__ __forceinline__ void thin_store_chunk(const uint32_t (&v)[64], float slope, uint4* tile, int lane,
                                                 __nv_bfloat16* dst, long long pix0, int ld, long long total_pix) {
    bias_act_pack<ACT>(v, nullptr, slope, tile, lane);
    __syncwarp();
#pragma unroll
    for (int i = 0; i < 8; ++i) {
        const int row = i * 4 + (lane >> 3), ch = lane & 7;
        const uint4 val = tile[row * 8 + (ch ^ (row & 7))];
        const long long pix = pix0 + row;
        if (pix < total_pix) *reinterpret_cast<uint4*>(dst + pix * ld + ch * 8) = val;
    }
    __syncwarp();
}

__device__ __forceinline__ void thin_store_dispatch(const uint32_t (&v)[64], int act, float slope, uint4* tile, int lane,
                                                    __nv_bfloat16* dst, long long pix0, int ld, long long total_pix) {
    if (act == PAI_ACT_LEAKY)
        thin_store_chunk<PAI_ACT_LEAKY>(v, slope, tile, lane, dst, pix0, ld, total_pix);
    else if (act == PAI_ACT_RELU)
        thin_store_chunk<PAI_ACT_RELU>(v, slope, tile, lane, dst, pix0, ld, total_pix);
    else if (act == PAI_ACT_TANH)
        thin_store_chunk<PAI_ACT_TANH>(v, slope, tile, lane, dst, pix0, ld, total_pix);
    else
        thin_store_chunk<PAI_ACT_NONE>(v, slope, tile, lane, dst, pix0, ld, total_pix);
}

static constexpr int kThinRing = 16;
static constexpr int kThinRowW = 256;

__device__ __forceinline__ void bulk_g2s(void* dst, const void* src, uint32_t bytes, uint64_t* bar) {
    asm volatile("cp.async.bulk.shared::cluster.global.mbarrier::complete_tx::bytes [%0], [%1], %2, [%3];" ::"r"(
                     smem_u32(dst)),
                 "l"(src), "r"(bytes), "r"(smem_u32(bar))
                 : "memory");
}

template <int CIN, bool STREAM>
__global__ void __launch_bounds__(kThinFpropThreads, 1) thin_conv_fprop_kernel(const ThinFpropParams p) {
    pdl_launch_dependents();
    pdl_wait();
    extern __shared__ uint8_t smem_raw[];
    __shared__ ThinPipe ps;
    __shared__ uint64_t ring_full[kThinRing], ring_empty[kThinRing];
    __shared__ uint4 stage_buf[8][32 * 8];
    uint8_t* smem = reinterpret_cast<uint8_t*>((reinterpret_cast<uintptr_t>(smem_raw) + 1023) & ~uintptr_t(1023));
    uint8_t* sA = smem;
    uint8_t* sB = smem + 2 * 16384;
    float* ring = reinterpret_cast<float*>(sB + (size_t)p.cout * 128);
    const int warp = threadIdx.x >> 5, lane = threadIdx.x & 31;
    const uint32_t acc_cols = tmem_cols_for(p.cout);
    const long long t_begin = STREAM ? (long long)p.tiles * blockIdx.x / gridDim.x : (long long)blockIdx.x;
    const long long t_step = STREAM ? 1 : (long long)gridDim.x;
    const int t_count = STREAM ? (int)((long long)p.tiles * (blockIdx.x + 1) / gridDim.x - t_begin)
                               : (int)(((long long)p.tiles - blockIdx.x + gridDim.x - 1) / gridDim.x);

    for (int i = threadIdx.x; i < p.cout * 8; i += kThinFpropThreads) {
        const int row = i >> 3, c = i & 7;
        *reinterpret_cast<uint4*>(sB + sw128_off(row, c)) = __ldg(reinterpret_cast<const uint4*>(p.w) + i);
    }
    if (p.bias != nullptr) {
        __syncthreads();
        for (int co = threadIdx.x; co < p.cout; co += kThinFpropThreads) {
            const float b = __ldg(p.bias + co);
            const __nv_bfloat16 hi = __float2bfloat16_rn(b);
            const __nv_bfloat16 lo = __float2bfloat16_rn(b - __bfloat162float(hi));
// ... 220 lines not shown
                }
                {
                    TROLE_T0();
                    mbar_wait(&ps.a_full[s], ph);
                    TROLE_ADD(w_a);
                }
                tc_fence_after();
                const uint64_t da0 = umma_desc_kmajor_sw128(smem_u32(sA + s * 16384));
                const uint32_t td = tmem_base + s * acc_cols;
                umma_bf16_ss(td, da0, db0, idesc, 0);
                if (CIN == 2) umma_bf16_acc(td, da0 + 2, db0 + 2, idesc);
                if (p.bias != nullptr) umma_bf16_acc(td, da0 + 2 * CIN, db0 + 2 * CIN, idesc);
                umma_commit(&ps.a_empty[s]);
                umma_commit(&ps.acc_full[s]);
            }
#ifdef PAI_PROFILE_ROLES
            if (blockIdx.x == 0)
                printf("[thin roles] mma: total %lld cyc, waiting for a drained accumulator %lld, for a built A tile %lld\n",
                       clock64() - tstart, w_acc, w_a);
#endif
        }
    } else if (warp >= 8) {
        const int q = warp & 3;
        const int g = (warp - 8) >> 2;
        const int r = q * 32 + lane;
        uint4* tile_buf = stage_buf[warp - 8];
        int k = 0;
        long long ep_wait = 0, ep_work = 0;
        (void)ep_wait, (void)ep_work;
        for (int i = g; i < t_count; i += 2, ++k) {
            const long long tile = t_begin + (long long)i * t_step;
            {
                TROLE_T0();
                mbar_wait(&ps.acc_full[g], (uint32_t)(k & 1));
                TROLE_ADD(ep_wait);
            }
#ifdef PAI_PROFILE_ROLES
            const long long tw0 = clock64();
#endif
            tc_fence_after();
            const uint32_t td = tmem_base + g * acc_cols + ((uint32_t)(q * 32) << 16);
            for (int c0 = 0; c0 < p.cout; c0 += 64) {
                uint32_t v[64];
#pragma unroll
                for (int j = 0; j < 4; ++j)
                    tmem_ld_16(td + (uint32_t)(c0 + 16 * j), *reinterpret_cast<uint32_t(*)[16]>(&v[16 * j]));
                tmem_ld_wait();
                if (c0 + 64 >= p.cout) {
                    tc_fence_before();
                    __syncwarp();
                    if (lane == 0) mbar_arrive_relaxed(&ps.acc_empty[g]);
                }
                const long long pix0 = tile * 128 + q * 32;
                thin_store_dispatch(v, p.act1, p.slope, tile_buf, lane, p.out1 + c0, pix0, p.ld1, p.total_pix);
                if (p.out2 != nullptr)
                    thin_store_dispatch(v, p.act2, p.slope, tile_buf, lane, p.out2 + c0, pix0, p.ld2, p.total_pix);
            }
#ifdef PAI_PROFILE_ROLES
            ep_work += clock64() - tw0;
#endif
        }
#ifdef PAI_PROFILE_ROLES
        if (blockIdx.x == 0 && lane == 0 && (warp == 8 || warp == 12))
            printf("[thin roles] epilogue warp %d: waiting for a full accumulator %lld cyc, working %lld cyc over %d tiles\n", warp,
                   ep_wait, ep_work, k);
#endif
    }
    tc_fence_before();
    __syncthreads();
    if (warp == 4) {
        tc_fence_after();
        tmem_dealloc(tmem_base, 2 * acc_cols);
    }
}

static constexpr int kThinWgradThreads = 256;
static constexpr int kThinWgradStages = 6;

struct ThinWgradParams {
    const float* p0;
    const float* p1;
    int n, ih, iw, oh, ow;
    int c;
    long long blocks;
    int blocks_per_row;
    float* dw;
    FastDiv fd_bpr, fd_oh;
};

struct __align__(8) ThinWgradPipe {
    uint64_t full[kThinWgradStages], empty[kThinWgradStages], acc_full;
    uint32_t tmem_base;
};

template <int CIN>
__global__ void __launch_bounds__(kThinWgradThreads, 1)
thin_wgrad_kernel(const __grid_constant__ CUtensorMap tm_u, const ThinWgradParams p) {
    pdl_launch_dependents();
    constexpr int N = 16 * CIN;
    constexpr uint32_t kABytes = 2 * 8192, kBBytes = 4096, kStage = kABytes + kBBytes;
    extern __shared__ uint8_t smem_raw[];
    __shared__ ThinWgradPipe ps;
    uint8_t* smem = reinterpret_cast<uint8_t*>((reinterpret_cast<uintptr_t>(smem_raw) + 1023) & ~uintptr_t(1023));
    const int warp = threadIdx.x >> 5, lane = threadIdx.x & 31;
    const long long b_begin = p.blocks * blockIdx.x / gridDim.x, b_end = p.blocks * (blockIdx.x + 1) / gridDim.x;

    if (warp == 0 && lane == 0) tma_prefetch_desc(&tm_u);
// ... 300 lines not shown
                        o += (rgt ? ring[sp][8][b + 1] : 0.f) + ring[sp][10][b];
                    }
                    if (p.act == PAI_ACT_TANH) e = tanhf(e), o = tanhf(o);
                    *reinterpret_cast<float2*>(out_img + (size_t)(2 * a - 1) * (2 * kPlaneW) + 2 * b) = make_float2(e, o);
                }
            }
            r = (long long)img * p.h + a_hi;
        }
    }
    tc_fence_before();
    __syncthreads();
    if (warp == 2) {
        tc_fence_after();
        tmem_dealloc(tmem_base, 32);
    }
}

__global__ void __launch_bounds__(256)
col2im4x4s1_kernel(const float* __restrict__ P, int ldp, int n, int h, int w, float* __restrict__ out) {
    pdl_launch_dependents();
    pdl_wait();
    const int oh = h - 1, ow = w - 1;
    const int total = n * oh * ow;
    for (int idx = blockIdx.x * 256 + threadIdx.x; idx < total; idx += gridDim.x * 256) {
        const int ox = idx % ow;
        const int r = idx / ow;
        const int oy = r % oh, img = r / oh;
        const float* base = P + (size_t)img * h * w * ldp;
        float s = 0.f;
#pragma unroll
        for (int ky = 0; ky < 4; ++ky) {
            const int iy = oy - 1 + ky;
            if (iy < 0 || iy >= h) continue;
#pragma unroll
            for (int kx = 0; kx < 4; ++kx) {
                const int ix = ox - 1 + kx;
                if (ix >= 0 && ix < w) s += __ldg(base + ((size_t)iy * w + ix) * ldp + ky * 4 + kx);
            }
        }
        out[idx] = s;
    }
}

static bool aligned16p(const void* p) { return (reinterpret_cast<uintptr_t>(p) & 15) == 0; }

}

using namespace pai;

extern "C" {

int pai_thin_conv4x4s2_fprop(const float* plane0, const float* plane1, int cin, int n, int ih, int iw,
                             const void* w_packed, int cout, const float* bias, void* out1, int ld1, int act1, void* out2,
                             int ld2, int act2, float slope, void* stream_) {
    PAI_REQUIRE(plane0 && w_packed && out1 && (cin == 1 || (cin == 2 && plane1)), "pai_thin_conv4x4s2_fprop: bad planes / cin=%d", cin);
    PAI_REQUIRE(ih % 2 == 0 && iw % 2 == 0 && n > 0, "pai_thin_conv4x4s2_fprop: even image sizes (got %dx%d)", ih, iw);
    PAI_REQUIRE(cout >= 64 && cout <= 256 && cout % 64 == 0, "pai_thin_conv4x4s2_fprop: cout (%d) must be 64..256, %% 64", cout);
    PAI_REQUIRE(ld1 % 8 == 0 && aligned16p(out1) && aligned16p(w_packed) && (out2 == nullptr || (ld2 % 8 == 0 && aligned16p(out2))) &&
                    (bias == nullptr || aligned16p(bias)),
                "pai_thin_conv4x4s2_fprop: outputs / weights / bias must be 16 B aligned with ld %% 8 == 0");
    ThinFpropParams p;
    p.p0 = plane0, p.p1 = plane1, p.n = n, p.ih = ih, p.iw = iw, p.oh = ih / 2, p.ow = iw / 2;
    p.w = (const __nv_bfloat16*)w_packed, p.cout = cout, p.bias = bias;
    p.out1 = (__nv_bfloat16*)out1, p.ld1 = ld1, p.act1 = act1, p.out2 = (__nv_bfloat16*)out2, p.ld2 = ld2, p.act2 = act2;
    p.slope = slope;
    p.total_pix = (long long)n * p.oh * p.ow;
    PAI_REQUIRE(p.total_pix < (1LL << 31) - 128, "pai_thin_conv4x4s2_fprop: tensor too large");
    p.tiles = (int)((p.total_pix + 127) / 128);
    p.fd_ow = make_fastdiv(p.ow), p.fd_oh = make_fastdiv(p.oh);
    const int dev = current_device(), sms = persistent_ctas(dev);
    if (sms < 0) return -1;
    const bool stream = iw == kThinRowW && (reinterpret_cast<uintptr_t>(plane0) & 15) == 0 &&
                        (plane1 == nullptr || (reinterpret_cast<uintptr_t>(plane1) & 15) == 0) && getenv("PAI_THIN_GATHER") == nullptr;
    const size_t smem = 2 * 16384 + (size_t)cout * 128 + (stream ? (size_t)kThinRing * cin * 2 * kThinRowW * 4 : 0) + 1024;
    static DeviceOnce once;
    if (once.need(dev)) {
        const int cap = 2 * 16384 + 256 * 128 + kThinRing * 2 * 2 * kThinRowW * 4 + 1024;
        PAI_CUDA_OK(cudaFuncSetAttribute(thin_conv_fprop_kernel<1, false>, cudaFuncAttributeMaxDynamicSharedMemorySize, cap));
        PAI_CUDA_OK(cudaFuncSetAttribute(thin_conv_fprop_kernel<2, false>, cudaFuncAttributeMaxDynamicSharedMemorySize, cap));
        PAI_CUDA_OK(cudaFuncSetAttribute(thin_conv_fprop_kernel<1, true>, cudaFuncAttributeMaxDynamicSharedMemorySize, cap));
        PAI_CUDA_OK(cudaFuncSetAttribute(thin_conv_fprop_kernel<2, true>, cudaFuncAttributeMaxDynamicSharedMemorySize, cap));
        once.mark(dev);
    }
    const int grid = p.tiles < sms ? p.tiles : sms;
    cudaStream_t st = (cudaStream_t)stream_;
    if (cin == 1 && stream)
        PAI_CUDA_OK(launch_pdl(thin_conv_fprop_kernel<1, true>, dim3((unsigned)grid), dim3(kThinFpropThreads), smem, st, 1, p));
    else if (cin == 1)
        PAI_CUDA_OK(launch_pdl(thin_conv_fprop_kernel<1, false>, dim3((unsigned)grid), dim3(kThinFpropThreads), smem, st, 1, p));
    else if (stream)
        PAI_CUDA_OK(launch_pdl(thin_conv_fprop_kernel<2, true>, dim3((unsigned)grid), dim3(kThinFpropThreads), smem, st, 1, p));
    else
        PAI_CUDA_OK(launch_pdl(thin_conv_fprop_kernel<2, false>, dim3((unsigned)grid), dim3(kThinFpropThreads), smem, st, 1, p));
    PAI_CUDA_OK(cudaGetLastError());
    return 0;
}

int pai_thin_conv4x4s2_wgrad(const void* u, int u_ld, int c, const float* plane0, const float* plane1, int cin, int n,
                             int ih, int iw, float* dw, void* stream) {
    PAI_REQUIRE(u && plane0 && dw && (cin == 1 || (cin == 2 && plane1)), "pai_thin_conv4x4s2_wgrad: bad planes / cin=%d", cin);
    PAI_REQUIRE((c == 64 || c == 128) && u_ld % 8 == 0 && u_ld >= c && aligned16p(u),
                "pai_thin_conv4x4s2_wgrad: c (%d) must be 64 or 128, u 16 B aligned", c);
    PAI_REQUIRE(ih % 2 == 0 && iw % 128 == 0 && (reinterpret_cast<uintptr_t>(plane0) & 15) == 0 &&
                    (plane1 == nullptr || (reinterpret_cast<uintptr_t>(plane1) & 15) == 0),
                "pai_thin_conv4x4s2_wgrad: image width (%d) must be a multiple of 128, planes 16 B aligned", iw);
    ThinWgradParams p;
    p.p0 = plane0, p.p1 = plane1, p.n = n, p.ih = ih, p.iw = iw, p.oh = ih / 2, p.ow = iw / 2, p.c = c, p.dw = dw;
    const long long pixels = (long long)n * p.oh * p.ow;
    PAI_REQUIRE(pixels < (1LL << 31), "pai_thin_conv4x4s2_wgrad: tensor too large");
    p.blocks = pixels / 64;
    p.blocks_per_row = p.ow / 64;
    p.fd_bpr = make_fastdiv(p.blocks_per_row), p.fd_oh = make_fastdiv(p.oh);
    CUtensorMap tm_u;
    uint64_t dims[2] = {(uint64_t)c, (uint64_t)pixels};
    uint64_t str[1] = {(uint64_t)u_ld * 2};
    uint32_t box[2] = {64, 64};
    int rc = encode_tmap_bf16(&tm_u, u, 2, dims, str, box);
    if (rc) return rc;
    const int dev = current_device(), sms = persistent_ctas(dev);
    if (sms < 0) return -1;
// ... 70 lines not shown
```

thesis-pai-reconstruction_b200/pai_b200/engine.py:

```python
from __future__ import annotations

import os
from typing import List, Optional

import torch

from . import dp, ops
from .ops import ACT_LEAKY, ACT_NONE, ACT_RELU, ACT_TANH

BN_EPS, BN_MOMENTUM, SLOPE = 1e-5, 0.1, 0.2
FUSE_BN_STATS = os.environ.get("PAI_NO_BN_FUSION") is None
FUSE_ACT_BWD = os.environ.get("PAI_NO_ACT_BWD_FUSION") is None
THIN_DIRECT = os.environ.get("PAI_NO_THIN_DIRECT") is None


class _PackCache:

    def get(self, tag: str, p: torch.Tensor, fn):
        store = p.__dict__.setdefault("_pai_packs", {})
        stamp = (p._version, p.data_ptr())
        ent = store.get(tag)
        if ent is None or ent[0] != stamp:
            with torch.no_grad():
                ent = (stamp, fn(p.detach()))
# ... 574 lines not shown
    @staticmethod
    def forward(ctx, spec: UnetSpec, training: bool, x: torch.Tensor, *params):
        need = any(ctx.needs_input_grad[3:])
        if ctx.needs_input_grad[2]:
            raise RuntimeError("pai_b200: the fused generator node has no gradient w.r.t. its input image "
                               "(the reference never asks for one, models/wrapper.py:117-162); detach x")
        y, saved = unet_forward(spec, x, training, save=need)
        ctx.spec, ctx.saved, ctx.training = spec, saved, training
        return y

    @staticmethod
    def backward(ctx, grad_y):
        if ctx.saved is None:
            raise RuntimeError("pai_b200: generator backward requested but the forward ran without a graph")
        if not ctx.training and any(b is not None for b in ctx.spec.enc_bns + ctx.spec.dec_bns):
            raise RuntimeError("pai_b200: gradients through an eval-mode BatchNorm generator are not implemented "
                               "(the reference only differentiates in train mode, models/wrapper.py:117-162)")
        grads = unet_backward(ctx.spec, ctx.saved, grad_y)
        ctx.saved = None
        need = ctx.needs_input_grad[3:]
        return (None, None, None) + tuple(g if nd else None for g, nd in zip(grads, need))


class DiscSpec:
    def __init__(self, convs):
        self.convs = convs
        self.ch = [c.weight.shape[0] for c in convs]
        cin0 = convs[0].weight.shape[1]
        if cin0 % 2 or not (2 <= cin0 <= CARRIER):
            raise RuntimeError("pai_b200: the PatchGAN's first conv reads cat([x, y]) of two images with the same number "
                               f"of channels (at most {CARRIER} together); it has {cin0} inputs")
        self.img_ch = cin0 // 2
        if self.ch[-1] != 1 or convs[-1].bias is not None:
            raise RuntimeError("pai_b200: unexpected PatchGAN head")

    def params(self):
        ps = []
        for c in self.convs[:-1]:
            ps += [c.weight, c.bias]
        ps.append(self.convs[-1].weight)
        return ps


def disc_forward(spec: DiscSpec, x: torch.Tensor, y: torch.Tensor, save: bool):
    n, _, h, w = x.shape
    dev = x.device
    if not (x.is_cuda and y.is_cuda and spec.convs[0].weight.is_cuda):
        raise RuntimeError("pai_b200: the PatchGAN runs on the B200 kernels only: inputs and parameters must be CUDA tensors "
                           "(there is no CPU or PyTorch fallback)")
    if x.shape[1] != spec.img_ch or y.shape[1] != spec.img_ch:
        raise RuntimeError(f"pai_b200: this PatchGAN takes two {spec.img_ch}-channel images, got {x.shape[1]} and {y.shape[1]}")
    c0 = spec.convs[0]
    xycol = xyc = px = py = None
    if spec.img_ch == 1:
        px = x.contiguous().float().view(n, h, w)
        py = y.contiguous().float().view(n, h, w)
    if spec.img_ch != 1:
        xyc = _carrier(x.float(), y.float())
        hcur = ops.conv4x4_fprop(xyc, _carrier_in_pack(c0.weight), spec.ch[0], stride=2, bias=c0.bias.detach(), act=ACT_LEAKY,
                                 slope=SLOPE)
    elif THIN_DIRECT and spec.ch[0] <= 256:
        hcur = _bf16(n, h // 2, w // 2, spec.ch[0], device=dev)
        ops.thin_conv_fprop([px, py], _thin_in_pack(c0.weight), spec.ch[0], c0.bias.detach(), hcur, ACT_LEAKY, slope=SLOPE)
    else:
        xycol = ops.im2col4x4([px, py], h // 2, w // 2, stride=2)
        hcur = ops.pointwise_gemm(xycol, _thin_in_pack(c0.weight), spec.ch[0], bias=c0.bias.detach(), act=ACT_LEAKY,
                                  slope=SLOPE, k_valid=32)
    hs = [hcur]
    for k in range(1, len(spec.convs) - 1):
        c = spec.convs[k]
        hcur = ops.conv4x4_fprop(hcur, _fprop_pack(c.weight), spec.ch[k], stride=2, bias=c.bias.detach(),
                                 act=ACT_LEAKY, slope=SLOPE)
        hs.append(hcur)
    head = spec.convs[-1]
    if THIN_DIRECT:
        part = ops.pointwise_gemm(hcur, _head_fprop_pack(head.weight), 16, out_f32=True)
        logits = ops.col2im4x4s1(part)
        nb, lh, lw = logits.shape
    else:
        logits = ops.conv4x4_fprop(hcur, _fprop_pack(head.weight), 1, stride=1, out_f32=True)
        nb, lh, lw, _ = logits.shape
    logits = logits.view(nb, 1, lh, lw)
    if not save:
        return logits, None
    s = _Saved()
    s.px, s.py, s.hs, s.xycol, s.xyc, s.hw = px, py, hs, xycol, xyc, (h, w)
    return logits, s


def disc_backward(spec: DiscSpec, s: _Saved, g_logits: torch.Tensor, need_params: bool, need_y: bool):
    dev = g_logits.device
    n, _, lh, lw = g_logits.shape
    g = g_logits.contiguous().float().view(n, lh, lw)
    K = len(spec.convs)
    head = spec.convs[-1]
    h_last = s.hs[-1]
    c_last = h_last.shape[3]
    grads = [None] * (2 * (K - 1) + 1)
    gcol = ops.im2col4x4([g], h_last.shape[1], h_last.shape[2], stride=1, flip=True)
    if need_params:
        dwh = ops.pointwise_wgrad(h_last, gcol)[:, :16]
        grads[-1] = dwh.reshape(1, c_last, 4, 4)
    dh = ops.pointwise_gemm(gcol, _head_dgrad_pack(head.weight), c_last, k_valid=16)
    fused = None
    for k in range(K - 2, -1, -1):
        conv = spec.convs[k]
        hk = s.hs[k]
        ck = hk.shape[3]
        if fused is not None:
            d_pre, sums = fused
            fused = None
        else:
            d_pre = _bf16(*hk.shape, device=dev)
            sums = ops.act_bwd(hk, dh, ACT_LEAKY, None, ACT_NONE, d_pre, slope=SLOPE)
        if k > 0:
            if need_params:
                grads[2 * k] = ops.wgrad_finish(ops.conv4x4_wgrad(s.hs[k - 1], d_pre, stride=2))
                dp.allreduce_async(grads[2 * k])
                grads[2 * k + 1] = sums[:ck].clone()
            cprev = s.hs[k - 1].shape[3]
            if FUSE_ACT_BWD and ops.bn_fusable(s.hs[k - 1].numel() // cprev, cprev):
                d_next, part = ops.conv4x4_dgrad_act(d_pre, _dgrad_pack(conv.weight), cprev, s.hs[k - 1], slope=SLOPE,
                                                     want_colsum=need_params)
                fused = (d_next, part.sum(0) if part is not None else None)
            else:
                dh = ops.convT4x4s2_fprop(d_pre, _dgrad_pack(conv.weight), cprev)
        elif s.xyc is not None:
            h, w = s.hw
            if need_params:
                dw0 = ops.wgrad_finish(ops.conv4x4_wgrad(s.xyc, d_pre, stride=2))
                grads[0] = dw0[:, :2 * spec.img_ch].contiguous()
                grads[1] = sums[:ck].clone()
            gy = None
            if need_y:
                gyc = ops.convT4x4s2_fprop(d_pre, _carrier_in_dgrad_pack(conv.weight), CARRIER, out_f32=True)
                gy = gyc[..., spec.img_ch:2 * spec.img_ch].permute(0, 3, 1, 2).contiguous()
        else:
            h, w = s.hw
            if need_params:
                if THIN_DIRECT and ops.thin_wgrad_ok(d_pre, [s.px, s.py]):
                    dw0 = ops.thin_conv_wgrad(d_pre, [s.px, s.py])
                else:
                    xycol = s.xycol if s.xycol is not None else ops.im2col4x4([s.px, s.py], h // 2, w // 2, stride=2)
                    dw0 = ops.pointwise_wgrad(d_pre, xycol)
                grads[0] = dw0[:, :32].reshape(ck, 4, 4, 2).permute(0, 3, 1, 2)
                grads[1] = sums[:ck].clone()
            gy = None
            if need_y:
                if THIN_DIRECT and ops.thin_plane_ok(d_pre):
                    gy = ops.thin_convT_plane(d_pre, _thin_in_dgrad_pack(conv.weight, 1)).view(n, 1, h, w)
                else:
                    part = ops.pointwise_gemm(d_pre, _thin_in_dgrad_pack(conv.weight, 1), 16, out_f32=True)
                    gy = ops.col2im4x4s2(part).view(n, 1, h, w)
    dp.finish_async()
    return grads, gy


class DiscFunction(torch.autograd.Function):
    @staticmethod
    def forward(ctx, spec: DiscSpec, x, y, *params):
        need_params = any(ctx.needs_input_grad[3:])
        need_y = ctx.needs_input_grad[2]
        if ctx.needs_input_grad[1]:
            raise RuntimeError("pai_b200: the fused PatchGAN node has no gradient w.r.t. its first (conditioning) input "
                               "x (models/wrapper.py:126-128,147 only differentiate w.r.t. the prediction y); detach x")
        logits, saved = disc_forward(spec, x, y, save=need_params or need_y)
        ctx.spec, ctx.saved, ctx.need_params, ctx.need_y = spec, saved, need_params, need_y
        return logits

    @staticmethod
    def backward(ctx, g_logits):
        grads, gy = disc_backward(ctx.spec, ctx.saved, g_logits, ctx.need_params, ctx.need_y)
        ctx.saved = None
        need = ctx.needs_input_grad[3:]
        return (None, None, gy) + tuple(g if nd else None for g, nd in zip(grads, need))
```

thesis-pai-reconstruction_b200/pai_b200/lib.py:

```python
from __future__ import annotations

import contextlib
import ctypes
import os

_HERE = os.path.dirname(os.path.abspath(__file__))
LIB_PATH = os.environ.get("PAI_LIB_PATH") or os.path.join(_HERE, "libpai_b200.so")

c_int, c_float, c_void_p, c_ll = ctypes.c_int, ctypes.c_float, ctypes.c_void_p, ctypes.c_longlong

SIGNATURES = {
    "pai_version": [],
    "pai_reserve_sms": [c_int],
    "pai_conv4x4_fprop": [c_void_p, c_int, c_int, c_int, c_int, c_int, c_void_p, c_int, c_int, c_int, c_void_p,
                          c_int, c_float, c_void_p, c_int, c_int, c_int, c_void_p, c_void_p],
    "pai_convT4x4s2_fprop": [c_void_p, c_int, c_int, c_int, c_int, c_int, c_void_p, c_int, c_int, c_void_p, c_int,
                             c_float, c_void_p, c_int, c_int, c_int, c_void_p, c_void_p],
    "pai_conv4x4_wgrad": [c_void_p, c_int, c_int, c_int, c_int, c_int, c_void_p, c_int, c_int, c_int, c_void_p,
                          c_int, c_void_p],
    "pai_convT4x4s2_wgrad": [c_void_p, c_int, c_int, c_int, c_int, c_int, c_void_p, c_int, c_int, c_void_p, c_int,
                             c_void_p],
    "pai_ssim_psnr_fwd": [c_void_p, c_void_p, c_int, c_int, c_int, c_int, c_int, c_void_p, c_void_p, c_void_p,
                          c_void_p, c_void_p],
    "pai_ssim_psnr_bwd": [c_void_p, c_void_p, c_int, c_int, c_int, c_int, c_int, c_void_p, c_void_p, c_void_p,
                          c_void_p, c_void_p],
    "pai_bn_stats": [c_void_p, c_ll, c_int, c_int, c_void_p, c_void_p],
    "pai_bn_finalize": [c_void_p, c_ll, c_int, c_void_p, c_void_p, c_float, c_float, c_int, c_void_p, c_void_p,
                        c_void_p, c_void_p],
    "pai_bn_apply_act": [c_void_p, c_ll, c_int, c_int, c_void_p, c_void_p, c_int, c_int, c_void_p, c_int, c_int,
                         c_float, c_void_p],
    "pai_bn_bwd_reduce": [c_void_p, c_ll, c_int, c_int, c_void_p, c_void_p, c_int, c_int, c_void_p, c_int, c_int,
                          c_float, c_void_p, c_void_p],
    "pai_bn_bwd_apply": [c_void_p, c_ll, c_int, c_int, c_void_p, c_void_p, c_int, c_int, c_void_p, c_int, c_int,
                         c_float, c_void_p, c_void_p, c_void_p, c_int, c_void_p],
    "pai_act_bwd": [c_void_p, c_ll, c_int, c_int, c_void_p, c_int, c_int, c_void_p, c_int, c_int, c_float, c_void_p,
                    c_void_p, c_int, c_void_p],
    "pai_colsum": [c_void_p, c_ll, c_int, c_int, c_void_p, c_void_p],
    "pai_bn_small_fwd": [c_void_p, c_ll, c_int, c_int, c_void_p, c_void_p, c_float, c_float, c_void_p, c_void_p, c_void_p,
                         c_void_p, c_int, c_int, c_void_p, c_int, c_int, c_float, c_void_p, c_int, c_void_p],
    "pai_bn_small_bwd": [c_void_p, c_ll, c_int, c_int, c_void_p, c_void_p, c_int, c_int, c_void_p, c_int, c_int, c_float,
                         c_void_p, c_int, c_void_p, c_void_p, c_void_p, c_int, c_void_p],
    "pai_smallc_conv_fprop": [c_void_p, c_void_p, c_int, c_int, c_int, c_int, c_int, c_int, c_int, c_int, c_void_p,
                              c_void_p, c_int, c_void_p, c_int, c_int, c_void_p, c_int, c_int, c_float, c_void_p],
    "pai_smallc_conv_wgrad": [c_void_p, c_int, c_int, c_void_p, c_void_p, c_int, c_int, c_int, c_int, c_int, c_int,
                              c_int, c_int, c_void_p, c_void_p],
    "pai_im2col4x4": [c_void_p, c_void_p, c_int, c_int, c_int, c_int, c_int, c_int, c_int, c_int, c_void_p, c_void_p],
    "pai_pointwise_gemm": [c_void_p, c_ll, c_int, c_int, c_void_p, c_int, c_int, c_void_p, c_int, c_float, c_void_p,
                           c_int, c_int, c_void_p, c_int, c_int, c_int, c_int, c_void_p],
    "pai_pointwise_wgrad": [c_void_p, c_ll, c_int, c_int, c_void_p, c_int, c_int, c_void_p, c_int, c_void_p],
    "pai_col2im4x4s2": [c_void_p, c_int, c_int, c_int, c_int, c_void_p, c_int, c_void_p, c_void_p],
    "pai_conv3x3_fprop": [c_void_p, c_int, c_int, c_int, c_int, c_int, c_void_p, c_int, c_int, c_void_p, c_int, c_float,
                          c_void_p, c_int, c_int, c_int, c_void_p, c_void_p],
    "pai_conv3x3_wgrad": [c_void_p, c_int, c_int, c_int, c_int, c_int, c_void_p, c_int, c_int, c_void_p, c_void_p],
    "pai_maxpool2_fwd": [c_void_p, c_int, c_int, c_int, c_int, c_int, c_void_p, c_int, c_void_p],
    "pai_maxpool2_bwd": [c_void_p, c_int, c_int, c_int, c_int, c_int, c_void_p, c_int, c_void_p, c_int, c_void_p],
    "pai_upsample2_fwd": [c_void_p, c_int, c_int, c_int, c_int, c_int, c_void_p, c_int, c_void_p],
    "pai_upsample2_bwd": [c_void_p, c_int, c_int, c_int, c_int, c_int, c_void_p, c_int, c_void_p],
    "pai_add_act": [c_void_p, c_int, c_void_p, c_int, c_ll, c_int, c_int, c_float, c_void_p, c_int, c_void_p],
    "pai_scale_rows_fwd": [c_void_p, c_int, c_void_p, c_ll, c_int, c_int, c_void_p, c_int, c_void_p],
    "pai_scale_rows_bwd": [c_void_p, c_int, c_void_p, c_void_p, c_int, c_ll, c_int, c_int, c_void_p, c_int, c_void_p,
                           c_void_p],
    "pai_conv_plane_to_wide": [c_void_p, c_int, c_int, c_int, c_int, c_int, c_int, c_void_p, c_void_p, c_int, c_int,
                               c_float, c_void_p, c_int, c_void_p],
    "pai_conv_wide_to_plane": [c_void_p, c_int, c_int, c_int, c_int, c_int, c_int, c_int, c_void_p, c_void_p, c_int,
                               c_void_p, c_void_p],
    "pai_conv_plane_wide_wgrad": [c_void_p, c_void_p, c_int, c_int, c_int, c_int, c_int, c_int, c_int, c_int, c_void_p,
                                  c_void_p],
    "pai_gconv4_3x3_fprop": [c_void_p, c_int, c_int, c_int, c_int, c_int, c_void_p, c_void_p, c_void_p, c_int, c_void_p],
    "pai_gconv4_3x3_wgrad": [c_void_p, c_int, c_void_p, c_int, c_int, c_int, c_int, c_int, c_void_p, c_void_p],
    "pai_subsample2": [c_void_p, c_int, c_int, c_int, c_int, c_int, c_void_p, c_int, c_int, c_void_p],
    "pai_layernorm_fwd": [c_void_p, c_ll, c_int, c_void_p, c_void_p, c_float, c_void_p, c_void_p, c_void_p, c_void_p],
    "pai_layernorm_bwd": [c_void_p, c_void_p, c_ll, c_int, c_void_p, c_void_p, c_void_p, c_void_p, c_void_p, c_void_p,
                          c_void_p],
    "pai_gelu_fwd": [c_void_p, c_ll, c_void_p, c_void_p],
    "pai_gelu_bwd": [c_void_p, c_void_p, c_ll, c_void_p, c_void_p],
    "pai_attn_fwd": [c_void_p, c_int, c_int, c_int, c_int, c_void_p, c_void_p, c_void_p],
    "pai_attn_bwd": [c_void_p, c_void_p, c_int, c_int, c_int, c_int, c_void_p, c_void_p, c_void_p, c_void_p],
    "pai_dropout_mask": [c_void_p, c_int, c_ll, c_float, c_void_p, c_void_p],
    "pai_attn_fwd_dropout": [c_void_p, c_int, c_int, c_int, c_int, c_void_p, c_int, c_float, c_void_p, c_void_p, c_void_p],
    "pai_attn_bwd_dropout": [c_void_p, c_void_p, c_int, c_int, c_int, c_int, c_void_p, c_int, c_float, c_void_p, c_void_p,
                             c_void_p, c_void_p],
    "pai_add_dropout_layernorm_fwd": [c_void_p, c_void_p, c_ll, c_int, c_void_p, c_int, c_float, c_void_p, c_void_p,
                                      c_float, c_void_p, c_void_p, c_void_p, c_void_p, c_void_p],
    "pai_layernorm_bwd_dropout": [c_void_p, c_void_p, c_ll, c_int, c_void_p, c_void_p, c_void_p, c_void_p, c_int, c_float,
                                  c_void_p, c_void_p, c_void_p, c_void_p, c_void_p],
    "pai_gelu_dropout_fwd": [c_void_p, c_ll, c_void_p, c_int, c_float, c_void_p, c_void_p],
    "pai_gelu_dropout_bwd": [c_void_p, c_void_p, c_ll, c_void_p, c_int, c_float, c_void_p, c_void_p],
    "pai_adam_pack_conv4x4": [c_void_p, c_void_p, c_void_p, c_void_p, c_int, c_int, c_float, c_float, c_float, c_float,
                              c_float, c_void_p, c_void_p, c_int, c_void_p, c_void_p],
    "pai_scale_channels": [c_void_p, c_int, c_void_p, c_int, c_ll, c_int, c_void_p, c_int, c_void_p],
    "pai_conv4x4_fprop_bnstats": [c_void_p, c_int, c_int, c_int, c_int, c_int, c_void_p, c_int, c_int, c_int, c_void_p,
                                  c_void_p, c_int, c_int, c_void_p, c_int, c_void_p],
    "pai_convT4x4s2_fprop_bnstats": [c_void_p, c_int, c_int, c_int, c_int, c_int, c_void_p, c_int, c_int, c_void_p,
                                     c_void_p, c_int, c_int, c_void_p, c_int, c_void_p],
    "pai_conv4x4_dgrad_act": [c_void_p, c_int, c_int, c_int, c_int, c_int, c_void_p, c_int, c_int, c_void_p, c_float,
                              c_void_p, c_int, c_int, c_void_p, c_int, c_void_p],
    "pai_bn_finalize_partials": [c_void_p, c_int, c_ll, c_int, c_void_p, c_void_p, c_float, c_float, c_int, c_void_p,
                                 c_void_p, c_void_p, c_void_p],
    "pai_wgrad_finish": [c_void_p, c_ll, c_void_p, c_int, c_void_p],
    "pai_adam_prepare": [c_void_p, c_float, c_float, c_float, c_void_p, c_void_p],
    "pai_check_conv2d_f32": [c_void_p, c_int, c_int, c_int, c_int, c_void_p, c_int, c_int, c_int, c_int, c_void_p, c_int,
                             c_float, c_int, c_void_p, c_void_p],
    "pai_check_batchnorm_f32": [c_void_p, c_int, c_int, c_int, c_void_p, c_void_p, c_void_p, c_void_p, c_int, c_float,
                                c_float, c_void_p, c_void_p],
    "pai_check_act_f32": [c_void_p, c_ll, c_int, c_float, c_void_p, c_void_p],
    "pai_check_conv2d_wgrad_f32": [c_void_p, c_int, c_int, c_int, c_int, c_void_p, c_int, c_int, c_int, c_int, c_int, c_float,
                                   c_int, c_void_p, c_void_p, c_void_p],
    "pai_check_batchnorm_bwd_f32": [c_void_p, c_void_p, c_int, c_int, c_int, c_void_p, c_float, c_void_p, c_void_p, c_void_p,
                                    c_void_p],
    "pai_check_act_bwd_f32": [c_void_p, c_void_p, c_ll, c_int, c_float, c_void_p, c_void_p],
    "pai_thin_conv4x4s2_fprop": [c_void_p, c_void_p, c_int, c_int, c_int, c_int, c_void_p, c_int, c_void_p, c_void_p, c_int,
                                 c_int, c_void_p, c_int, c_int, c_float, c_void_p],
    "pai_thin_conv4x4s2_wgrad": [c_void_p, c_int, c_int, c_void_p, c_void_p, c_int, c_int, c_int, c_int, c_void_p, c_void_p],
    "pai_thin_convT4x4s2_plane": [c_void_p, c_int, c_int, c_int, c_int, c_int, c_void_p, c_void_p, c_int, c_void_p, c_void_p],
    "pai_conv4x4_fprop_dual": [c_void_p, c_int, c_int, c_int, c_int, c_int, c_void_p, c_int, c_int, c_int, c_void_p, c_int,
                               c_float, c_void_p, c_int, c_void_p, c_int, c_int, c_int, c_void_p],
    "pai_to_uint8": [c_void_p, c_ll, c_void_p, c_void_p],
    "pai_afmhot_u8": [c_void_p, c_int, c_ll, c_void_p, c_void_p],
    "pai_col2im4x4s1": [c_void_p, c_int, c_int, c_int, c_int, c_void_p, c_void_p],
    "pai_resize_aa_normalize_u8": [c_void_p, c_int, c_int, c_int, c_int, c_int, c_int, c_int, c_void_p, c_void_p],
    "pai_ema_multi": [c_int, c_void_p, c_void_p, c_void_p, c_float, c_void_p],
    "pai_adam_pack_conv4x4_multi": [c_int, c_void_p, c_void_p, c_void_p, c_void_p, c_void_p, c_void_p, c_void_p, c_void_p,
                                    c_void_p, c_float, c_float, c_float, c_float, c_float, c_void_p, c_void_p],
    "pai_adam_multi": [c_int, c_void_p, c_void_p, c_void_p, c_void_p, c_void_p, c_float, c_float, c_float, c_float,
                       c_float, c_void_p, c_void_p],
}
RESTYPES = {"pai_ssim_bwd_workspace_bytes": (ctypes.c_longlong, [c_int, c_int, c_int]),
            "pai_bn_small_ok": (c_int, [c_ll, c_int, c_int])}

_lib = None
launches = 0


def load() -> ctypes.CDLL:
    global _lib
    if _lib is None:
        if not os.path.exists(LIB_PATH):
            raise RuntimeError(
                f"{LIB_PATH} is missing: build it with thesis-pai-reconstruction_b200/csrc/build.sh "
                "(or __graft_entry__.build()); there is no CPU or PyTorch fallback")
        lib = ctypes.CDLL(LIB_PATH)
        lib.pai_last_error.restype = ctypes.c_char_p
        lib.pai_last_error.argtypes = []
        for name, args in SIGNATURES.items():
            fn = getattr(lib, name)
            fn.argtypes = args
            fn.restype = c_int
        for name, (res, args) in RESTYPES.items():
            fn = getattr(lib, name)
            fn.argtypes = args
            fn.restype = res
        _lib = lib
    return _lib


def on_device(t):
    import torch
    return torch.cuda.device(t.device) if t.is_cuda else contextlib.nullcontext()


def call(name: str, *args, kernels: int = 1) -> None:
    global launches
    lib = load()
    rc = getattr(lib, name)(*args)
    if rc != 0:
# ... 3 lines not shown
```

thesis-pai-reconstruction_b200/pai_b200/ops.py:

```python
from __future__ import annotations

import ctypes
import os

import torch

from . import lib

ACT_NONE, ACT_LEAKY, ACT_RELU, ACT_TANH = 0, 1, 2, 3
BN_SMALL_OFF = os.environ.get("PAI_NO_BN_SMALL", "0") == "1"
_T_K = ((1, 3), (0, 2))


_prof = None


def profile_start():
    global _prof
    _prof = []


def profile_stop():
    global _prof
    out, _prof = _prof, None
# ... 76 lines not shown
class zero_pool:

    def __init__(self, device):
        on = device.type == "cuda" and os.environ.get("PAI_NO_ZERO_POOL", "0") != "1"
        self.pool = _zero_pools.setdefault((device.type, device.index), _ZeroPool()) if on else None
        self.device = device

    def __enter__(self):
        pl = self.pool
        if pl is None:
            return self
        pl.depth += 1
        if pl.depth == 1:
            pl.cursor = pl.demand = 0
            pl.buf = torch.zeros(pl.capacity, dtype=torch.float32, device=self.device) if pl.capacity else None
        return self

    def __exit__(self, *exc):
        pl = self.pool
        if pl is None:
            return False
        pl.depth -= 1
        if pl.depth == 0:
            pl.capacity, pl.buf = pl.demand, None
        return False


def zeros_f32(*shape, device) -> torch.Tensor:
    pl = _zero_pools.get((device.type, device.index))
    n = 1
    for d in shape:
        n *= int(d)
    if pl is None or pl.depth == 0 or n > _ZeroPool.MAX_ELEMS or n == 0:
        return torch.zeros(*shape, dtype=torch.float32, device=device)
    padded = (n + 63) & ~63
    pl.demand += padded
    if pl.buf is None or pl.cursor + padded > pl.buf.numel():
        return torch.zeros(*shape, dtype=torch.float32, device=device)
    out = pl.buf[pl.cursor:pl.cursor + n].view(*shape)
    pl.cursor += padded
    return out


SPLITK_MAX_PIXELS = 74 * 128


def _splitk_ws(pixels: int, cout: int, device):
    if pixels > SPLITK_MAX_PIXELS or cout < 16:
        return None
    return zeros_f32(pixels, cout, device=device)


def conv4x4_fprop(x, w_packed, cout, stride=2, bias=None, act=ACT_NONE, slope=0.2, out=None, out_f32=False,
                  n_tile=0):
    n, h, w, cin, ld = _nhwc(x)
    cp = w_packed.shape[0]
    ho, wo = (h // 2, w // 2) if stride == 2 else (h - 1, w - 1)
    if out is None:
        out = torch.empty(n, ho, wo, cout, dtype=torch.float32 if out_f32 else torch.bfloat16, device=x.device)
    on, oh, ow, oc, old = _nhwc(out)
    assert (on, oh, ow, oc) == (n, ho, wo, cout)
    ws = _splitk_ws(n * ho * wo, cout, x.device)
    _igemm_call("pai_conv4x4_fprop", 2.0 * n * ho * wo * cout * 16 * cin, _ptr(x), n, h, w, cin, ld, _ptr(w_packed), cout, cp, stride, _ptr(bias), act,
             float(slope), _ptr(out), old, int(out.dtype == torch.float32), n_tile, _ptr(ws), _stream())
    return out


def conv4x4_fprop_dual(x, w_packed, cout, bias, out1, act1, out2, act2, slope=0.2):
    n, h, w, cin, ld = _nhwc(x)
    cp = w_packed.shape[0]
    assert tuple(out1.shape) == tuple(out2.shape) == (n, h // 2, w // 2, cout)
    _igemm_call("pai_conv4x4_fprop_dual", 2.0 * n * (h // 2) * (w // 2) * cout * 16 * cin, _ptr(x), n, h, w, cin, ld,
                _ptr(w_packed), cout, cp, 2, _ptr(bias), act1, float(slope), _ptr(out1), _nhwc(out1)[4], _ptr(out2),
                _nhwc(out2)[4], act2, 0, _stream())


def to_uint8(x):
    x = x.contiguous().float()
    out = torch.empty(x.shape, dtype=torch.uint8, device=x.device)
    lib.call("pai_to_uint8", _ptr(x), x.numel(), _ptr(out), _stream())
    return out


def afmhot_uint8(img):
    img = img.contiguous().float()
    n, _, h, w = img.shape
    out = torch.empty(n, 3, h, w, dtype=torch.uint8, device=img.device)
    lib.call("pai_afmhot_u8", _ptr(img), n, h * w, _ptr(out), _stream())
    return out


BN_PART_ROWS = 160


def bn_fusable(pixels: int, cout: int) -> bool:
    return pixels > SPLITK_MAX_PIXELS and cout % 64 == 0


def conv4x4_fprop_bnstats(x, w_packed, cout, bias=None):
    n, h, w, cin, ld = _nhwc(x)
    cp = w_packed.shape[0]
    out = torch.empty(n, h // 2, w // 2, cout, dtype=torch.bfloat16, device=x.device)
    part = zeros_f32(BN_PART_ROWS, 2 * cout, device=x.device)
    _igemm_call("pai_conv4x4_fprop_bnstats", 2.0 * n * (h // 2) * (w // 2) * cout * 16 * cin, _ptr(x), n, h, w, cin, ld,
                _ptr(w_packed), cout, cp, 2, _ptr(bias), _ptr(out), cout, 0, _ptr(part), BN_PART_ROWS, _stream())
    return out, part


def convT4x4s2_fprop_bnstats(x, w_packed, cout, bias=None):
    n, h, w, cin, ld = _nhwc(x)
    cp = w_packed.shape[1]
    out = torch.empty(n, 2 * h, 2 * w, cout, dtype=torch.bfloat16, device=x.device)
    part = zeros_f32(BN_PART_ROWS, 2 * cout, device=x.device)
    _igemm_call("pai_convT4x4s2_fprop_bnstats", 2.0 * n * h * w * cout * 16 * cin, _ptr(x), n, h, w, cin, ld,
                _ptr(w_packed), cout, cp, _ptr(bias), _ptr(out), cout, 0, _ptr(part), BN_PART_ROWS, _stream())
    return out, part


def conv4x4_dgrad_act(gy, w_packed_dgrad, cin, saved_act, slope=0.2, want_colsum=True):
    n, h, w, cout, ld = _nhwc(gy)
    cp = w_packed_dgrad.shape[1]
    sn, sh, sw, sc, sld = _nhwc(saved_act)
    assert (sn, sh, sw, sc) == (n, 2 * h, 2 * w, cin) and sld == cin
    out = torch.empty(n, 2 * h, 2 * w, cin, dtype=torch.bfloat16, device=gy.device)
    part = zeros_f32(BN_PART_ROWS, 2 * cin, device=gy.device) if want_colsum else None
    _igemm_call("pai_conv4x4_dgrad_act", 2.0 * n * h * w * cin * 16 * cout, _ptr(gy), n, h, w, cout, ld,
                _ptr(w_packed_dgrad), cin, cp, _ptr(saved_act), float(slope), _ptr(out), cin, 0, _ptr(part), BN_PART_ROWS,
                _stream())
    return out, part


def convT4x4s2_fprop(x, w_packed, cout, bias=None, act=ACT_NONE, slope=0.2, out=None, out_f32=False, n_tile=0):
    n, h, w, cin, ld = _nhwc(x)
    cp = w_packed.shape[1]
    if out is None:
        out = torch.empty(n, 2 * h, 2 * w, cout, dtype=torch.float32 if out_f32 else torch.bfloat16, device=x.device)
    on, oh, ow, oc, old = _nhwc(out)
    assert (on, oh, ow, oc) == (n, 2 * h, 2 * w, cout)
    ws = _splitk_ws(4 * n * h * w, cout, x.device)
    _igemm_call("pai_convT4x4s2_fprop", 2.0 * n * h * w * cout * 16 * cin, _ptr(x), n, h, w, cin, ld, _ptr(w_packed), cout, cp, _ptr(bias), act,
             float(slope), _ptr(out), old, int(out.dtype == torch.float32), n_tile, _ptr(ws), _stream())
    return out


def conv4x4_wgrad(x, gy, stride=2, dw=None, splitk=0):
    n, h, w, cin, ld = _nhwc(x)
    gn, gh, gw, cout, gld = _nhwc(gy)
    if dw is None:
        dw = torch.zeros(16, cout, cin, dtype=torch.float32, device=x.device)
    _igemm_call("pai_conv4x4_wgrad", 2.0 * gn * gh * gw * cout * 16 * cin, _ptr(x), n, h, w, cin, ld, _ptr(gy), cout, gld, stride, _ptr(dw), splitk,
             _stream())
    return dw


def convT4x4s2_wgrad(x, gy, dw=None, splitk=0):
    n, h, w, cin, ld = _nhwc(x)
    gn, gh, gw, cout, gld = _nhwc(gy)
    if dw is None:
        dw = torch.zeros(16, cin, cout, dtype=torch.float32, device=x.device)
    _igemm_call("pai_convT4x4s2_wgrad", 2.0 * n * h * w * cout * 16 * cin, _ptr(x), n, h, w, cin, ld, _ptr(gy), cout, gld, _ptr(dw), splitk, _stream())
    return dw


def dropout2d_mask(n: int, c: int, p: float, device) -> torch.Tensor:
    keep = torch.bernoulli(torch.full((n, c), 1.0 - p, dtype=torch.float32, device=device))
    return keep.mul_(1.0 / (1.0 - p))


def scale_channels(x, mask, out=None):
    n, h, w, c, ld = _nhwc(x)
    assert mask.shape == (n, c) and mask.dtype == torch.float32 and mask.is_contiguous()
    if out is None:
        out = torch.empty(n, h, w, c, dtype=torch.bfloat16, device=x.device)
    lib.call("pai_scale_channels", _ptr(x), ld, _ptr(mask), n, h * w, c, _ptr(out), _nhwc(out)[4], _stream())
    return out


def wgrad_finish(dw: torch.Tensor) -> torch.Tensor:
    _, a, b = dw.shape
    grad = torch.empty(a, b, 4, 4, dtype=torch.float32, device=dw.device)
# ... 131 lines not shown
    _, ih, iw = p0.shape
    dw = torch.zeros(c, 16, len(planes), dtype=torch.float32, device=a.device)
    lib.call("pai_smallc_conv_wgrad", _ptr(a), lda, c, _ptr(p0), _ptr(p1), len(planes), n, ih, iw, oh, ow, stride,
             int(flip), _ptr(dw), _stream())
    return dw


def im2col4x4(planes, oh, ow, stride=2, flip=False):
    p0 = planes[0]
    p1 = planes[1] if len(planes) > 1 else None
    n, ih, iw = p0.shape
    col = torch.empty(n, oh, ow, 64, dtype=torch.bfloat16, device=p0.device)
    lib.call("pai_im2col4x4", _ptr(p0), _ptr(p1), len(planes), n, ih, iw, oh, ow, stride, int(flip), _ptr(col),
             _stream())
    return col


def pointwise_gemm(x, w_packed, cout, bias=None, act=ACT_NONE, slope=0.2, out=None, out_f32=False, out2=None,
                   act2=ACT_NONE, n_tile=0, k_valid=0):
    m, cin, ld = _mat(x)
    cp = w_packed.shape[0]
    if out is None:
        out = torch.empty(*x.shape[:-1], cout, dtype=torch.float32 if out_f32 else torch.bfloat16, device=x.device)
    mo, co, old = _mat(out)
    assert (mo, co) == (m, cout)
    old2 = 0
    if out2 is not None:
        m2, c2, old2 = _mat(out2)
        assert (m2, c2) == (m, cout)
    _igemm_call("pai_pointwise_gemm", 2.0 * m * cin * cout, _ptr(x), m, cin, ld, _ptr(w_packed), cout, cp, _ptr(bias),
                act, float(slope), _ptr(out), old, int(out.dtype == torch.float32), _ptr(out2), old2, act2, n_tile,
                k_valid, _stream())
    return out


def pointwise_wgrad(u, s, splitk=0):
    m, cu, uld = _mat(u)
    ms, cs, sld = _mat(s)
    assert ms == m
    dw = torch.zeros(cu, cs, dtype=torch.float32, device=u.device)
    _igemm_call("pai_pointwise_wgrad", 2.0 * m * cu * cs, _ptr(u), m, cu, uld, _ptr(s), cs, sld, _ptr(dw), splitk,
                _stream())
    return dw


def col2im4x4s2(p, bias=None, act=ACT_NONE):
    n, h, w, c = p.shape
    assert p.dtype == torch.float32 and p.stride(3) == 1 and c >= 16
    out = torch.empty(n, 2 * h, 2 * w, dtype=torch.float32, device=p.device)
    lib.call("pai_col2im4x4s2", _ptr(p), p.stride(2), n, h, w, _ptr(bias), act, _ptr(out), _stream())
    return out


def thin_conv_fprop(planes, w_packed, cout, bias, out1, act1=ACT_NONE, out2=None, act2=ACT_NONE, slope=0.2):
    p0 = planes[0]
    p1 = planes[1] if len(planes) > 1 else None
    n, ih, iw = p0.shape
    assert p0.is_contiguous() and p0.dtype == torch.float32 and (p1 is None or (p1.is_contiguous() and p1.shape == p0.shape))
    on, oh, ow, oc, ld1 = _nhwc(out1)
    assert (on, oh, ow, oc) == (n, ih // 2, iw // 2, cout) and tuple(w_packed.shape) == (cout, 64)
    ld2 = 0
    if out2 is not None:
        assert tuple(out2.shape) == (n, ih // 2, iw // 2, cout)
        ld2 = _nhwc(out2)[4]
    _igemm_call("pai_thin_conv4x4s2_fprop", 2.0 * n * (ih // 2) * (iw // 2) * cout * 16 * len(planes), _ptr(p0), _ptr(p1),
                len(planes), n, ih, iw, _ptr(w_packed), cout, _ptr(bias), _ptr(out1), ld1, act1, _ptr(out2), ld2, act2,
                float(slope), _stream())
    return out1


def thin_wgrad_ok(u, planes) -> bool:
    return u.shape[3] in (64, 128) and planes[0].shape[2] % 128 == 0


def thin_conv_wgrad(u, planes):
    n, oh, ow, c, uld = _nhwc(u)
    p0 = planes[0]
    p1 = planes[1] if len(planes) > 1 else None
    pn, ih, iw = p0.shape
    assert (pn, ih, iw) == (n, 2 * oh, 2 * ow) and p0.is_contiguous() and p0.dtype == torch.float32
    dw = torch.zeros(c, 16 * len(planes), dtype=torch.float32, device=u.device)
    _igemm_call("pai_thin_conv4x4s2_wgrad", 2.0 * n * oh * ow * c * 16 * len(planes), _ptr(u), uld, c, _ptr(p0), _ptr(p1),
                len(planes), n, ih, iw, _ptr(dw), _stream())
    return dw


def thin_plane_ok(x) -> bool:
    return x.shape[2] == 128 and x.shape[3] % 64 == 0 and x.shape[3] <= 256


def thin_convT_plane(x, w_taps, bias=None, act=ACT_NONE):
    n, h, w, c, ld = _nhwc(x)
    assert tuple(w_taps.shape) == (16, c) and w_taps.is_contiguous()
    out = torch.empty(n, 2 * h, 2 * w, dtype=torch.float32, device=x.device)
    _igemm_call("pai_thin_convT4x4s2_plane", 2.0 * n * h * w * c * 16, _ptr(x), n, h, w, c, ld, _ptr(w_taps), _ptr(bias),
                act, _ptr(out), _stream())
    return out


def col2im4x4s1(p):
    n, h, w, c = p.shape
    assert p.dtype == torch.float32 and p.stride(3) == 1 and c >= 16
    out = torch.empty(n, h - 1, w - 1, dtype=torch.float32, device=p.device)
    lib.call("pai_col2im4x4s1", _ptr(p), p.stride(2), n, h, w, _ptr(out), _stream())
    return out


def pack_conv1x1_weight(w: torch.Tensor) -> torch.Tensor:
    cout, cin = w.shape[0], w.shape[1]
    out = torch.zeros(padded_cout(cout), cin, dtype=torch.bfloat16, device=w.device)
    out[:cout].copy_(w.reshape(cout, cin))
    return out


def pack_conv1x1_weight_t(w: torch.Tensor) -> torch.Tensor:
    cout, cin = w.shape[0], w.shape[1]
    out = torch.zeros(padded_cout(cin), cout, dtype=torch.bfloat16, device=w.device)
    out[:cin].copy_(w.reshape(cout, cin).t())
    return out

# ... 313 lines not shown
```

Before: 9132.

## Save LeakyReLU sign bitmasks in forward and gate dgrad with them

Forward LeakyReLU convolutions now write a packed 64-bit sign mask per 64 channels alongside the bf16 output. The fused dgrad+activation-backward kernel reads these bits with L1 prefetch and __ldg instead of TMA-loading the full bf16 saved activation through an mbarrier. This cuts backward-pass memory traffic and removes the mask barrier machinery. In exchange, split-K is disabled for those forward convs and every masked epilogue now waits on the store group.

```diff
diff --git a/include/pai_b200.h b/include/pai_b200.h
--- a/include/pai_b200.h
+++ b/include/pai_b200.h
@@ -19,7 +19,7 @@
 
 int pai_conv4x4_fprop(const void* x, int n, int h, int w, int cin, int x_ld, const void* w_packed, int cout,
                       int cout_pad, int stride, const float* bias, int act, float slope, void* y, int y_ld,
-                      int y_f32, int n_tile, float* splitk_ws, void* stream);
+                      int y_f32, int n_tile, float* splitk_ws, void* act_bits, void* stream);
 
 int pai_conv4x4_fprop_dual(const void* x, int n, int h, int w, int cin, int x_ld, const void* w_packed, int cout,
                            int cout_pad, int stride, const float* bias, int act, float slope, void* y, int y_ld, void* y2,
@@ -35,7 +35,7 @@
                                  int cout_pad, const float* bias, void* y, int y_ld, int n_tile, float* bn_partials,
                                  int bn_rows, void* stream);
 int pai_conv4x4_dgrad_act(const void* gy, int n, int h, int w, int cout, int gy_ld, const void* w_packed_dgrad, int cin,
-                          int cin_pad, const void* saved_act, float slope, void* gx, int gx_ld, int n_tile,
+                          int cin_pad, const void* act_bits, float slope, void* gx, int gx_ld, int n_tile,
                           float* colsum_partials, int rows, void* stream);
 
 int pai_conv4x4_wgrad(const void* x, int n, int h, int w, int cin, int x_ld, const void* gy, int cout, int gy_ld,
@@ -66,6 +66,7 @@
 int pai_act_bwd(const void* x, long long m, int c, int ld, const void* g1, int ldg1, int act1, const void* g2, int ldg2,
                 int act2, float slope, float* sums2c, void* dx, int lddx, void* stream);
 int pai_colsum(const void* x, long long m, int c, int ld, float* sums2c, void* stream);
+int pai_act_sign_bits(const void* x, long long m, int c, int ld, void* bits, void* stream);
 int pai_bn_small_ok(long long m, int c, int operands);
 int pai_bn_small_fwd(const void* x, long long m, int c, int ld, const float* gamma, const float* beta, float eps,
                      float momentum, float* running_mean, float* running_var, float* scale_shift, void* out1, int ld1,
@@ -93,7 +94,7 @@
 
 int pai_thin_conv4x4s2_fprop(const float* plane0, const float* plane1, int cin, int n, int ih, int iw,
                              const void* w_packed, int cout, const float* bias, void* out1, int ld1, int act1, void* out2,
-                             int ld2, int act2, float slope, void* stream);
+                             int ld2, int act2, float slope, void* act_bits, void* stream);
 int pai_thin_conv4x4s2_wgrad(const void* u, int u_ld, int c, const float* plane0, const float* plane1, int cin, int n,
                              int ih, int iw, float* dw, void* stream);
 int pai_thin_convT4x4s2_plane(const void* x, int n, int h, int w, int c, int x_ld, const void* w_taps, const float* bias,
diff --git a/thesis-pai-reconstruction_b200/csrc/elementwise.cu b/thesis-pai-reconstruction_b200/csrc/elementwise.cu
--- a/thesis-pai-reconstruction_b200/csrc/elementwise.cu
+++ b/thesis-pai-reconstruction_b200/csrc/elementwise.cu
@@ -1,4 +1,5 @@
 #include "pai_common.cuh"
+#include "pai_epilogue.cuh"
 #include "pai_kernels.h"
 
 namespace pai {
@@ -735,6 +736,34 @@
     return 0;
 }
 
+__global__ void __launch_bounds__(256) act_sign_bits_kernel(const bf16* __restrict__ x, long long words, int c64, int ld,
+                                                            unsigned long long* __restrict__ bits) {
+    for (long long i = blockIdx.x * 256LL + threadIdx.x; i < words; i += (long long)gridDim.x * 256) {
+        const long long pix = i / c64;
+        const uint4* src = reinterpret_cast<const uint4*>(x + pix * ld + (i - pix * c64) * 64);
+        uint4 m[8];
+#pragma unroll
+        for (int q = 0; q < 8; ++q) m[q] = __ldg(src + q);
+        const uint32_t lo = pos_bits16(m[0], m[1]) | (pos_bits16(m[2], m[3]) << 16);
+        const uint32_t hi = pos_bits16(m[4], m[5]) | (pos_bits16(m[6], m[7]) << 16);
+        bits[i] = ((unsigned long long)hi << 32) | lo;
+    }
+}
+
+int pai_act_sign_bits(const void* x, long long m, int c, int ld, void* bits, void* stream) {
+    PAI_REQUIRE(x && bits && m > 0, "pai_act_sign_bits: null pointer / empty input");
+    PAI_REQUIRE(c % 64 == 0 && ld % 8 == 0 && ld >= c && (reinterpret_cast<uintptr_t>(x) & 15) == 0 &&
+                    (reinterpret_cast<uintptr_t>(bits) & 7) == 0,
+                "pai_act_sign_bits: needs c %% 64 == 0, 16 B aligned rows and 8 B aligned words (c=%d ld=%d)", c, ld);
+    const long long words = m * (c / 64);
+    long long blocks = (words + 255) / 256;
+    if (blocks > 148 * 16) blocks = 148 * 16;
+    act_sign_bits_kernel<<<(unsigned)blocks, 256, 0, (cudaStream_t)stream>>>((const bf16*)x, words, c / 64, ld,
+                                                                             (unsigned long long*)bits);
+    PAI_CUDA_OK(cudaGetLastError());
+    return 0;
+}
+
 int pai_colsum(const void* x, long long m, int c, int ld, float* sums2c, void* stream) {
     PAI_REQUIRE(x && sums2c && m > 0, "pai_colsum: null pointer / empty input");
     cudaStream_t st = (cudaStream_t)stream;
diff --git a/thesis-pai-reconstruction_b200/csrc/igemm.cu b/thesis-pai-reconstruction_b200/csrc/igemm.cu
--- a/thesis-pai-reconstruction_b200/csrc/igemm.cu
+++ b/thesis-pai-reconstruction_b200/csrc/igemm.cu
@@ -24,7 +24,6 @@
     uint64_t empty[kMaxStages];
     uint64_t acc_full[2];
     uint64_t acc_empty[2];
-    uint64_t mask_full[8];
     uint32_t tmem_base;
 };
 
@@ -69,8 +68,6 @@
             mbar_init(&ps.acc_full[a], 1);
             mbar_init(&ps.acc_empty[a], PAIR ? 16 : 8);
         }
-        if (MASKED)
-            for (int w = 0; w < 8; ++w) mbar_init(&ps.mask_full[w], 1);
         mbar_fence_init();
     }
     if (warp == 2) {
@@ -317,7 +314,6 @@
         const int n_out = p.out2 != nullptr ? 2 : 1;
         const int qpos = __shfl_sync(0xffffffffu, rpos, 0);
         uint4* tile = stage_buf[warp - 4];
-        uint32_t mask_phase = 0;
         const bool st_persist = fused || acc_n <= 128;
         float st_sum[8], st_sq[8];
 #pragma unroll
@@ -364,17 +360,14 @@
             const bool fast = p.tma_out && (n_tile & 63) == 0 && col0 + n_tile <= p.cout &&
                               (p.bias == nullptr || (reinterpret_cast<uintptr_t>(p.bias) & 15) == 0);
             const int bw0 = tw * p.bw + (qpos & 255), bh0 = th * p.bh + ((qpos >> 8) & 255), bn0 = tn * p.bn + (qpos >> 16);
-            const bool masked = MASKED && p.mask_src != nullptr && fast;
-            auto mask_load = [&](int c) {
-                __syncwarp();
-                if (lane == 0) {
-                    bulk_wait_group_read0();
-                    mbar_expect_tx(&ps.mask_full[warp - 4], 32 * 128);
-                    tma_load_4d(tile, &om.aux[fused ? c >> 6 : phase_idx], &ps.mask_full[warp - 4], col0 + (fused ? 0 : c),
-                                bw0, bh0, bn0);
-                }
+            const int bits_row = gn * p.bits_sn + gh * p.bits_sh + gw * p.bits_sw;
+            auto gate_ptr = [&](int c) {
+                return p.act_bits + bits_row + p.bits_phase_off[fused ? c >> 6 : phase_idx] + ((col0 + (fused ? 0 : c)) >> 6);
             };
-            if (masked && 64 * half < acc_n) mask_load(64 * half);
+            if (MASKED && fast && row_ok) {
+                if (64 * half < acc_n) prefetch_l1(gate_ptr(64 * half));
+                if (64 * (half + 2) < acc_n) prefetch_l1(gate_ptr(64 * (half + 2)));
+            }
             {
                 ROLE_T0();
                 mbar_wait(&ps.acc_full[a], acc_phase);
@@ -406,6 +399,7 @@
                     const int oc = fused ? 0 : c;
                     for (int which = 0; which < n_out; ++which, ++item) {
                         if ((item & 1) != half) continue;
+                        const uint64_t gate = MASKED && row_ok ? __ldg(gate_ptr(c)) : 0;
                         uint32_t v[64];
 #pragma unroll
                         for (int j = 0; j < 4; ++j)
@@ -414,14 +408,15 @@
                         if (item == last_item) release_acc();
                         const int act = which == 0 ? p.act : p.act2;
                         const float* bias_c = p.bias != nullptr ? p.bias + col0 + oc : nullptr;
-                        if (masked) {
-                            mbar_wait(&ps.mask_full[warp - 4], mask_phase);
-                            mask_phase ^= 1;
-                            mask_pack(v, p.mask_slope, tile, lane);
+                        if (lane == 0) bulk_wait_group_read0();
+                        __syncwarp();
+                        if (MASKED) {
+                            mask_pack(v, gate, p.mask_slope, tile, lane);
                         } else {
-                            if (lane == 0) bulk_wait_group_read0();
-                            __syncwarp();
-                            if (act == PAI_ACT_LEAKY)
+                            if (act == PAI_ACT_LEAKY && p.act_bits != nullptr) {
+                                const uint64_t bits = bias_act_pack<PAI_ACT_LEAKY, true>(v, bias_c, p.slope, tile, lane);
+                                if (which == 0 && row_ok) p.act_bits[bits_row + ((col0 + c) >> 6)] = bits;
+                            } else if (act == PAI_ACT_LEAKY)
                                 bias_act_pack<PAI_ACT_LEAKY>(v, bias_c, p.slope, tile, lane);
                             else if (act == PAI_ACT_RELU)
                                 bias_act_pack<PAI_ACT_RELU>(v, bias_c, p.slope, tile, lane);
@@ -433,7 +428,7 @@
                         fence_proxy_async_smem();
                         __syncwarp();
                         if (lane == 0) {
-                            tma_store_4d(which == 0 ? &om.out[fused ? c >> 6 : phase_idx] : &om.aux[0], tile, col0 + oc,
+                            tma_store_4d(which == 0 ? &om.out[fused ? c >> 6 : phase_idx] : &om.out2, tile, col0 + oc,
                                          bw0, bh0, bn0);
                             bulk_commit_group();
                         }
@@ -469,7 +464,6 @@
                                 reduce_add(cs, cq, col0 + oc);
                             }
                         }
-                        if (masked && c + 128 < acc_n) mask_load(c + 128);
                     }
                 }
             } else {
@@ -767,12 +761,16 @@
     } else {
         grid = (int)(total < num_sms ? total : num_sms);
     }
-    if (p.mask_src != nullptr)
+    if (p.act_bits != nullptr || p.masked) {
         PAI_REQUIRE(!p.out_f32 && p.splitk == 1 && !p.accumulate && (p.n_tile & 63) == 0 && p.cout % p.n_tile == 0 &&
-                        (p.cout & 7) == 0 && p.bias == nullptr && p.act == PAI_ACT_NONE && p.out2 == nullptr &&
-                        (reinterpret_cast<uintptr_t>(p.mask_src) & 15) == 0 && p.tma_out,
-                    "igemm fprop: the fused activation backward needs a plain bf16 output with 16 B aligned rows, "
+                        p.tma_out && p.out2 == nullptr && p.act_bits != nullptr && (reinterpret_cast<uintptr_t>(p.act_bits) & 7) == 0 &&
+                        (p.bias == nullptr || (reinterpret_cast<uintptr_t>(p.bias) & 15) == 0),
+                    "igemm fprop: activation sign words need a plain bf16 output with 16 B aligned rows, "
                     "cout %% 64 == 0 and no split-K (cout=%d n_tile=%d splitk=%d)", p.cout, p.n_tile, p.splitk);
+        PAI_REQUIRE(p.masked ? (p.bias == nullptr && p.act == PAI_ACT_NONE) : (p.act == PAI_ACT_LEAKY && phases == 1),
+                    "igemm fprop: activation sign words are read by a plain data gradient or written by a LeakyReLU "
+                    "convolution");
+    }
     if (p.bn_part != nullptr) {
         PAI_REQUIRE(!p.out_f32 && p.splitk == 1 && !p.accumulate && (p.n_tile & 63) == 0 && p.cout % p.n_tile == 0 &&
                         (p.cout & 7) == 0 && p.bn_rows >= grid,
@@ -781,11 +779,11 @@
     }
     const int cl = pair ? 2 : 1;
     const dim3 g((unsigned)grid), b(kFpropThreads);
-    if (pair && p.mask_src != nullptr)
+    if (pair && p.masked)
         PAI_CUDA_OK(launch_pdl(igemm_fprop_kernel<true, true>, g, b, smem, stream, cl, tm_a, tm_b, om, p));
     else if (pair)
         PAI_CUDA_OK(launch_pdl(igemm_fprop_kernel<true, false>, g, b, smem, stream, cl, tm_a, tm_b, om, p));
-    else if (p.mask_src != nullptr)
+    else if (p.masked)
         PAI_CUDA_OK(launch_pdl(igemm_fprop_kernel<false, true>, g, b, smem, stream, cl, tm_a, tm_b, om, p));
     else
         PAI_CUDA_OK(launch_pdl(igemm_fprop_kernel<false, false>, g, b, smem, stream, cl, tm_a, tm_b, om, p));
diff --git a/thesis-pai-reconstruction_b200/csrc/pai_api.cu b/thesis-pai-reconstruction_b200/csrc/pai_api.cu
--- a/thesis-pai-reconstruction_b200/csrc/pai_api.cu
+++ b/thesis-pai-reconstruction_b200/csrc/pai_api.cu
@@ -159,17 +159,23 @@
         int rc = map_out(&om->out[j], static_cast<const __nv_bfloat16*>(p.out) + p.out_phase_off[j], p.cout, p.gw, p.gh,
                          p.gn, p.out_sw, p.out_sh, p.out_sn, b);
         if (rc) return rc;
-        if (p.mask_src != nullptr) {
-            rc = map_out(&om->aux[j], static_cast<const __nv_bfloat16*>(p.mask_src) + p.out_phase_off[j], p.cout, p.gw,
-                         p.gh, p.gn, p.out_sw, p.out_sh, p.out_sn, b);
-            if (rc) return rc;
-        }
     }
     if (p.out2 != nullptr) {
-        int rc = map_out(&om->aux[0], p.out2, p.cout, p.gw, p.gh, p.gn, p.out2_sw, p.out2_sh, p.out2_sn, b);
+        int rc = map_out(&om->out2, p.out2, p.cout, p.gw, p.gh, p.gn, p.out2_sw, p.out2_sh, p.out2_sn, b);
         if (rc) return rc;
     }
     p.tma_out = 1;
+    return 0;
+}
+
+static int map_bits(IgemmFpropParams& p, uint64_t* bits, int nmaps, long long ld) {
+    const long long c64 = p.cout / 64;
+    PAI_REQUIRE(p.cout % 64 == 0 && (reinterpret_cast<uintptr_t>(bits) & 7) == 0,
+                "activation sign words need cout %% 64 == 0 (got %d) and an 8 B aligned buffer", p.cout);
+    PAI_REQUIRE(p.out_sn / ld * c64 * p.gn < (1LL << 31), "activation sign words: tensor too large");
+    p.act_bits = bits;
+    p.bits_sn = (int)(p.out_sn / ld * c64), p.bits_sh = (int)(p.out_sh / ld * c64), p.bits_sw = (int)(p.out_sw / ld * c64);
+    for (int j = 0; j < nmaps; ++j) p.bits_phase_off[j] = (int)(p.out_phase_off[j] / ld * c64);
     return 0;
 }
 
@@ -211,7 +217,7 @@
 static int conv4x4_fprop_impl(const void* x, int n, int h, int w, int cin, int x_ld, const void* w_packed, int cout,
                               int cout_pad, int stride, const float* bias, int act, float slope, void* y, int y_ld,
                               int y_f32, int n_tile, float* splitk_ws, float* bn_part, int bn_rows, void* stream,
-                              void* y2 = nullptr, int y2_ld = 0, int act2 = PAI_ACT_NONE) {
+                              void* y2 = nullptr, int y2_ld = 0, int act2 = PAI_ACT_NONE, void* act_bits = nullptr) {
     PAI_REQUIRE(x && w_packed && y, "pai_conv4x4_fprop: null pointer");
     PAI_REQUIRE(stride == 1 || stride == 2, "pai_conv4x4_fprop: stride must be 1 or 2 (got %d)", stride);
     PAI_REQUIRE(cin > 0 && cin % 64 == 0, "pai_conv4x4_fprop: cin must be a multiple of 64 (got %d)", cin);
@@ -235,6 +241,11 @@
     int rc = stride == 2 ? map_split(&tm_a, x, n, h, w, cin, b) : map_unit(&tm_a, x, n, h, w, cin, x_ld, b);
     if (rc) return rc;
     const int m_tiles = b.tiles_w * b.tiles_h * b.tiles_n;
+    if (act_bits != nullptr) {
+        PAI_REQUIRE(act == PAI_ACT_LEAKY && !y_f32 && cout == cout_pad && cout % 64 == 0,
+                    "pai_conv4x4_fprop: activation sign words need a LeakyReLU bf16 output with cout %% 64 == 0");
+        splitk_ws = nullptr;
+    }
     const int splitk = pick_splitk(splitk_ws, (long long)m_tiles * (cout_pad / n_tile), 16 * (cin / 64));
     const bool pair = igemm_fprop_use_pair(n_tile, m_tiles, cout_pad / n_tile, 1, splitk);
     uint64_t bd[2] = {(uint64_t)16 * cin, (uint64_t)cout_pad};
@@ -284,6 +295,10 @@
     }
     rc = map_outputs(&om, p, 1, b);
     if (rc) return rc;
+    if (act_bits != nullptr) {
+        rc = map_bits(p, static_cast<uint64_t*>(act_bits), 1, y_ld);
+        if (rc) return rc;
+    }
     return launch_igemm_fprop(tm_a, tm_b, om, p, m_tiles, cout_pad / n_tile, 1, (cudaStream_t)stream);
 }
 
@@ -297,9 +312,9 @@
 
 int pai_conv4x4_fprop(const void* x, int n, int h, int w, int cin, int x_ld, const void* w_packed, int cout,
                       int cout_pad, int stride, const float* bias, int act, float slope, void* y, int y_ld,
-                      int y_f32, int n_tile, float* splitk_ws, void* stream) {
+                      int y_f32, int n_tile, float* splitk_ws, void* act_bits, void* stream) {
     return conv4x4_fprop_impl(x, n, h, w, cin, x_ld, w_packed, cout, cout_pad, stride, bias, act, slope, y, y_ld, y_f32,
-                              n_tile, splitk_ws, nullptr, 0, stream);
+                              n_tile, splitk_ws, nullptr, 0, stream, nullptr, 0, PAI_ACT_NONE, act_bits);
 }
 int pai_conv4x4_fprop_bnstats(const void* x, int n, int h, int w, int cin, int x_ld, const void* w_packed, int cout,
                               int cout_pad, int stride, const float* bias, void* y, int y_ld, int n_tile,
@@ -312,7 +327,7 @@
 static int convT4x4s2_fprop_impl(const void* x, int n, int h, int w, int cin, int x_ld, const void* w_packed, int cout,
                                  int cout_pad, const float* bias, int act, float slope, void* y, int y_ld, int y_f32,
                                  int n_tile, float* splitk_ws, float* bn_part, int bn_rows, void* stream,
-                                 const void* mask_src = nullptr, float mask_slope = 0.f) {
+                                 const void* act_bits = nullptr, float mask_slope = 0.f) {
     PAI_REQUIRE(x && w_packed && y, "pai_convT4x4s2_fprop: null pointer");
     PAI_REQUIRE(cin > 0 && cin % 64 == 0, "pai_convT4x4s2_fprop: cin must be a multiple of 64 (got %d)", cin);
     PAI_REQUIRE(cout_pad % 16 == 0 && cout <= cout_pad, "pai_convT4x4s2_fprop: bad cout %d / cout_pad %d", cout, cout_pad);
@@ -354,7 +369,7 @@
                 }
     p.b_rows_per_phase = cout_pad;
     p.bn_part = bn_part, p.bn_rows = bn_rows;
-    p.mask_src = mask_src, p.mask_slope = mask_slope;
+    p.masked = act_bits != nullptr, p.mask_slope = mask_slope;
     const long long wo = 2LL * w;
     p.splitk = splitk;
     const long long ld = p.splitk > 1 ? cout : y_ld;
@@ -394,6 +409,10 @@
         p.bias = bias, p.act = act, p.slope = slope, p.out_f32 = 0, p.out = y;
         rc = map_outputs(&om, p, 4, b);
         if (rc) return rc;
+        if (act_bits != nullptr) {
+            rc = map_bits(p, const_cast<uint64_t*>(static_cast<const uint64_t*>(act_bits)), 4, ld);
+            if (rc) return rc;
+        }
         return launch_igemm_fprop(tm_a, tm_b, om, p, m_tiles, 1, 1, (cudaStream_t)stream);
     }
     if (p.splitk > 1) {
@@ -406,6 +425,10 @@
     p.bias = bias, p.act = act, p.slope = slope, p.out_f32 = y_f32, p.out = y;
     rc = map_outputs(&om, p, 4, b);
     if (rc) return rc;
+    if (act_bits != nullptr) {
+        rc = map_bits(p, const_cast<uint64_t*>(static_cast<const uint64_t*>(act_bits)), 4, ld);
+        if (rc) return rc;
+    }
     return launch_igemm_fprop(tm_a, tm_b, om, p, m_tiles, cout_pad / n_tile, 4, (cudaStream_t)stream);
 }
 
@@ -424,12 +447,12 @@
 }
 
 int pai_conv4x4_dgrad_act(const void* gy, int n, int h, int w, int cout, int gy_ld, const void* w_packed_dgrad, int cin,
-                          int cin_pad, const void* saved_act, float slope, void* gx, int gx_ld, int n_tile,
+                          int cin_pad, const void* act_bits, float slope, void* gx, int gx_ld, int n_tile,
                           float* colsum_partials, int rows, void* stream) {
-    PAI_REQUIRE(saved_act != nullptr, "pai_conv4x4_dgrad_act: null saved activation");
+    PAI_REQUIRE(act_bits != nullptr, "pai_conv4x4_dgrad_act: null sign words of the saved activation");
     PAI_REQUIRE(colsum_partials == nullptr || rows > 0, "pai_conv4x4_dgrad_act: bad partial-sum buffer");
     return convT4x4s2_fprop_impl(gy, n, h, w, cout, gy_ld, w_packed_dgrad, cin, cin_pad, nullptr, PAI_ACT_NONE, 0.f, gx,
-                                 gx_ld, 0, n_tile, nullptr, colsum_partials, rows, stream, saved_act, slope);
+                                 gx_ld, 0, n_tile, nullptr, colsum_partials, rows, stream, act_bits, slope);
 }
 
 static int wgrad_common(const void* u, int un, int uh, int uw, int cu, int u_ld, const void* s, int sh, int sw,
diff --git a/thesis-pai-reconstruction_b200/csrc/pai_common.cuh b/thesis-pai-reconstruction_b200/csrc/pai_common.cuh
--- a/thesis-pai-reconstruction_b200/csrc/pai_common.cuh
+++ b/thesis-pai-reconstruction_b200/csrc/pai_common.cuh
@@ -127,6 +127,8 @@
         "l"(reinterpret_cast<uint64_t>(map)), "r"(smem_u32(bar)), "r"(c0), "r"(c1), "r"(c2), "r"(c3), "r"(c4)
         : "memory");
 }
+__device__ __forceinline__ void prefetch_l1(const void* ptr) { asm volatile("prefetch.global.L1 [%0];" ::"l"(ptr)); }
+
 __device__ __forceinline__ void tma_prefetch_5d(const CUtensorMap* map, int c0, int c1, int c2, int c3, int c4) {
     asm volatile("cp.async.bulk.prefetch.tensor.5d.L2.global.tile [%0, {%1, %2, %3, %4, %5}];" ::"l"(
                      reinterpret_cast<uint64_t>(map)),
diff --git a/thesis-pai-reconstruction_b200/csrc/pai_epilogue.cuh b/thesis-pai-reconstruction_b200/csrc/pai_epilogue.cuh
--- a/thesis-pai-reconstruction_b200/csrc/pai_epilogue.cuh
+++ b/thesis-pai-reconstruction_b200/csrc/pai_epilogue.cuh
@@ -47,9 +47,16 @@
     if (ACT == PAI_ACT_TANH) return tanhf(v);
     return v;
 }
-template <int ACT>
-__device__ __forceinline__ void bias_act_pack(const uint32_t (&v)[64], const float* __restrict__ bias, float slope,
-                                              uint4* tile, int lane) {
+__device__ __forceinline__ uint32_t pos_pair(uint32_t w, int i) {
+    return __hgt2_mask(*reinterpret_cast<const __nv_bfloat162*>(&w), __float2bfloat162_rn(0.f)) &
+           ((1u << (2 * i)) | (1u << (17 + 2 * i)));
+}
+__device__ __forceinline__ uint32_t fold16(uint32_t y) { return (y & 0x5555u) | ((y >> 16) & 0xaaaau); }
+
+template <int ACT, bool BITS = false>
+__device__ __forceinline__ uint64_t bias_act_pack(const uint32_t (&v)[64], const float* __restrict__ bias, float slope,
+                                                  uint4* tile, int lane) {
+    uint32_t y = 0, half[2] = {0, 0};
 #pragma unroll
     for (int ch = 0; ch < 8; ++ch) {
         float f[8];
@@ -66,22 +73,35 @@
         for (int k = 0; k < 4; ++k) {
             __nv_bfloat162 h = __floats2bfloat162_rn(act_t<ACT>(f[2 * k], slope), act_t<ACT>(f[2 * k + 1], slope));
             w[k] = *reinterpret_cast<uint32_t*>(&h);
+            if (BITS) y |= pos_pair(w[k], 4 * (ch & 1) + k);
         }
         tile[lane * 8 + (ch ^ (lane & 7))] = make_uint4(w[0], w[1], w[2], w[3]);
+        if (BITS && (ch & 1)) {
+            half[ch >> 2] |= fold16(y) << (16 * ((ch >> 1) & 1));
+            y = 0;
+        }
     }
+    return ((uint64_t)half[1] << 32) | half[0];
 }
 
-__device__ __forceinline__ void mask_pack(const uint32_t (&v)[64], float slope, uint4* tile, int lane) {
+__device__ __forceinline__ uint32_t pos_bits16(const uint4& a, const uint4& b) {
+    const uint32_t w[8] = {a.x, a.y, a.z, a.w, b.x, b.y, b.z, b.w};
+    uint32_t y = 0;
+#pragma unroll
+    for (int i = 0; i < 8; ++i) y |= pos_pair(w[i], i);
+    return fold16(y);
+}
+
+__device__ __forceinline__ void mask_pack(const uint32_t (&v)[64], uint64_t bits, float slope, uint4* tile, int lane) {
+    const uint32_t lo = (uint32_t)bits, hi = (uint32_t)(bits >> 32);
 #pragma unroll
     for (int ch = 0; ch < 8; ++ch) {
-        const uint4 m = tile[lane * 8 + (ch ^ (lane & 7))];
-        const __nv_bfloat162* mh = reinterpret_cast<const __nv_bfloat162*>(&m);
+        const uint32_t b8 = ((ch < 4 ? lo : hi) >> (8 * (ch & 3))) & 0xffu;
         uint32_t w[4];
 #pragma unroll
         for (int k = 0; k < 4; ++k) {
-            const float2 mf = __bfloat1622float2(mh[k]);
-            const float a = __uint_as_float(v[8 * ch + 2 * k]) * (mf.x > 0.f ? 1.f : slope);
-            const float b = __uint_as_float(v[8 * ch + 2 * k + 1]) * (mf.y > 0.f ? 1.f : slope);
+            const float a = __uint_as_float(v[8 * ch + 2 * k]) * (((b8 >> (2 * k)) & 1u) ? 1.f : slope);
+            const float b = __uint_as_float(v[8 * ch + 2 * k + 1]) * (((b8 >> (2 * k + 1)) & 1u) ? 1.f : slope);
             __nv_bfloat162 h = __floats2bfloat162_rn(a, b);
             w[k] = *reinterpret_cast<uint32_t*>(&h);
         }
diff --git a/thesis-pai-reconstruction_b200/csrc/pai_kernels.h b/thesis-pai-reconstruction_b200/csrc/pai_kernels.h
--- a/thesis-pai-reconstruction_b200/csrc/pai_kernels.h
+++ b/thesis-pai-reconstruction_b200/csrc/pai_kernels.h
@@ -58,7 +58,10 @@
     int kmma;
     float* bn_part;
     int bn_rows;
-    const void* mask_src;
+    uint64_t* act_bits;
+    int bits_sn, bits_sh, bits_sw;
+    int bits_phase_off[4];
+    int masked;
     float mask_slope;
     int pair;
     int splitk;
@@ -68,7 +71,7 @@
 
 struct IgemmOutMaps {
     CUtensorMap out[4];
-    CUtensorMap aux[4];
+    CUtensorMap out2;
 };
 
 struct IgemmWgradParams {
diff --git a/thesis-pai-reconstruction_b200/csrc/thin.cu b/thesis-pai-reconstruction_b200/csrc/thin.cu
--- a/thesis-pai-reconstruction_b200/csrc/thin.cu
+++ b/thesis-pai-reconstruction_b200/csrc/thin.cu
@@ -27,6 +27,7 @@
     int ld1, act1;
     __nv_bfloat16* out2;
     int ld2, act2;
+    uint64_t* act_bits;
     float slope;
     long long total_pix;
     int tiles;
@@ -38,10 +39,10 @@
     uint32_t tmem_base;
 };
 
-template <int ACT>
-__device__ __forceinline__ void thin_store_chunk(const uint32_t (&v)[64], float slope, uint4* tile, int lane,
-                                                 __nv_bfloat16* dst, long long pix0, int ld, long long total_pix) {
-    bias_act_pack<ACT>(v, nullptr, slope, tile, lane);
+template <int ACT, bool BITS = false>
+__device__ __forceinline__ uint64_t thin_store_chunk(const uint32_t (&v)[64], float slope, uint4* tile, int lane,
+                                                     __nv_bfloat16* dst, long long pix0, int ld, long long total_pix) {
+    const uint64_t bits = bias_act_pack<ACT, BITS>(v, nullptr, slope, tile, lane);
     __syncwarp();
 #pragma unroll
     for (int i = 0; i < 8; ++i) {
@@ -51,6 +52,7 @@
         if (pix < total_pix) *reinterpret_cast<uint4*>(dst + pix * ld + ch * 8) = val;
     }
     __syncwarp();
+    return bits;
 }
 
 __device__ __forceinline__ void thin_store_dispatch(const uint32_t (&v)[64], int act, float slope, uint4* tile, int lane,
@@ -377,7 +379,13 @@
                     if (lane == 0) mbar_arrive_relaxed(&ps.acc_empty[g]);
                 }
                 const long long pix0 = tile * 128 + q * 32;
-                thin_store_dispatch(v, p.act1, p.slope, tile_buf, lane, p.out1 + c0, pix0, p.ld1, p.total_pix);
+                if (p.act_bits != nullptr) {
+                    const uint64_t bits = thin_store_chunk<PAI_ACT_LEAKY, true>(v, p.slope, tile_buf, lane, p.out1 + c0, pix0,
+                                                                                p.ld1, p.total_pix);
+                    if (pix0 + lane < p.total_pix) p.act_bits[((int)pix0 + lane) * (p.cout >> 6) + (c0 >> 6)] = bits;
+                } else {
+                    thin_store_dispatch(v, p.act1, p.slope, tile_buf, lane, p.out1 + c0, pix0, p.ld1, p.total_pix);
+                }
                 if (p.out2 != nullptr)
                     thin_store_dispatch(v, p.act2, p.slope, tile_buf, lane, p.out2 + c0, pix0, p.ld2, p.total_pix);
             }
@@ -784,7 +792,7 @@
 
 int pai_thin_conv4x4s2_fprop(const float* plane0, const float* plane1, int cin, int n, int ih, int iw,
                              const void* w_packed, int cout, const float* bias, void* out1, int ld1, int act1, void* out2,
-                             int ld2, int act2, float slope, void* stream_) {
+                             int ld2, int act2, float slope, void* act_bits, void* stream_) {
     PAI_REQUIRE(plane0 && w_packed && out1 && (cin == 1 || (cin == 2 && plane1)), "pai_thin_conv4x4s2_fprop: bad planes / cin=%d", cin);
     PAI_REQUIRE(ih % 2 == 0 && iw % 2 == 0 && n > 0, "pai_thin_conv4x4s2_fprop: even image sizes (got %dx%d)", ih, iw);
     PAI_REQUIRE(cout >= 64 && cout <= 256 && cout % 64 == 0, "pai_thin_conv4x4s2_fprop: cout (%d) must be 64..256, %% 64", cout);
@@ -795,9 +803,12 @@
     p.p0 = plane0, p.p1 = plane1, p.n = n, p.ih = ih, p.iw = iw, p.oh = ih / 2, p.ow = iw / 2;
     p.w = (const __nv_bfloat16*)w_packed, p.cout = cout, p.bias = bias;
     p.out1 = (__nv_bfloat16*)out1, p.ld1 = ld1, p.act1 = act1, p.out2 = (__nv_bfloat16*)out2, p.ld2 = ld2, p.act2 = act2;
+    PAI_REQUIRE(act_bits == nullptr || (act1 == PAI_ACT_LEAKY && (reinterpret_cast<uintptr_t>(act_bits) & 7) == 0),
+                "pai_thin_conv4x4s2_fprop: activation sign words need a LeakyReLU first output and an 8 B aligned buffer");
+    p.act_bits = (uint64_t*)act_bits;
     p.slope = slope;
     p.total_pix = (long long)n * p.oh * p.ow;
-    PAI_REQUIRE(p.total_pix < (1LL << 31) - 128, "pai_thin_conv4x4s2_fprop: tensor too large");
+    PAI_REQUIRE(p.total_pix * (act_bits != nullptr ? cout / 64 : 1) < (1LL << 31) - 128, "pai_thin_conv4x4s2_fprop: tensor too large");
     p.tiles = (int)((p.total_pix + 127) / 128);
     p.fd_ow = make_fastdiv(p.ow), p.fd_oh = make_fastdiv(p.oh);
     const int dev = current_device(), sms = persistent_ctas(dev);
diff --git a/thesis-pai-reconstruction_b200/pai_b200/engine.py b/thesis-pai-reconstruction_b200/pai_b200/engine.py
--- a/thesis-pai-reconstruction_b200/pai_b200/engine.py
+++ b/thesis-pai-reconstruction_b200/pai_b200/engine.py
@@ -650,17 +650,26 @@
         raise RuntimeError(f"pai_b200: this PatchGAN takes two {spec.img_ch}-channel images, got {x.shape[1]} and {y.shape[1]}")
     c0 = spec.convs[0]
     xycol = xyc = px = py = None
+    K = len(spec.convs)
+    bits = [None] * (K - 1)
+    if save and FUSE_ACT_BWD:
+        for k in range(K - 2):
+            hk, wk = h >> (k + 1), w >> (k + 1)
+            if ops.bn_fusable(n * hk * wk, spec.ch[k]):
+                bits[k] = ops.empty_act_bits(n, hk, wk, spec.ch[k], dev)
     if spec.img_ch == 1:
         px = x.contiguous().float().view(n, h, w)
         py = y.contiguous().float().view(n, h, w)
     if spec.img_ch != 1:
         xyc = _carrier(x.float(), y.float())
         hcur = ops.conv4x4_fprop(xyc, _carrier_in_pack(c0.weight), spec.ch[0], stride=2, bias=c0.bias.detach(), act=ACT_LEAKY,
-                                 slope=SLOPE)
+                                 slope=SLOPE, act_bits=bits[0])
     elif THIN_DIRECT and spec.ch[0] <= 256:
         hcur = _bf16(n, h // 2, w // 2, spec.ch[0], device=dev)
-        ops.thin_conv_fprop([px, py], _thin_in_pack(c0.weight), spec.ch[0], c0.bias.detach(), hcur, ACT_LEAKY, slope=SLOPE)
+        ops.thin_conv_fprop([px, py], _thin_in_pack(c0.weight), spec.ch[0], c0.bias.detach(), hcur, ACT_LEAKY, slope=SLOPE,
+                            act_bits=bits[0])
     else:
+        bits[0] = None
         xycol = ops.im2col4x4([px, py], h // 2, w // 2, stride=2)
         hcur = ops.pointwise_gemm(xycol, _thin_in_pack(c0.weight), spec.ch[0], bias=c0.bias.detach(), act=ACT_LEAKY,
                                   slope=SLOPE, k_valid=32)
@@ -668,7 +677,7 @@
     for k in range(1, len(spec.convs) - 1):
         c = spec.convs[k]
         hcur = ops.conv4x4_fprop(hcur, _fprop_pack(c.weight), spec.ch[k], stride=2, bias=c.bias.detach(),
-                                 act=ACT_LEAKY, slope=SLOPE)
+                                 act=ACT_LEAKY, slope=SLOPE, act_bits=bits[k])
         hs.append(hcur)
     head = spec.convs[-1]
     if THIN_DIRECT:
@@ -682,7 +691,7 @@
     if not save:
         return logits, None
     s = _Saved()
-    s.px, s.py, s.hs, s.xycol, s.xyc, s.hw = px, py, hs, xycol, xyc, (h, w)
+    s.px, s.py, s.hs, s.bits, s.xycol, s.xyc, s.hw = px, py, hs, bits, xycol, xyc, (h, w)
     return logits, s
 
 
@@ -717,9 +726,9 @@
                 dp.allreduce_async(grads[2 * k])
                 grads[2 * k + 1] = sums[:ck].clone()
             cprev = s.hs[k - 1].shape[3]
-            if FUSE_ACT_BWD and ops.bn_fusable(s.hs[k - 1].numel() // cprev, cprev):
-                d_next, part = ops.conv4x4_dgrad_act(d_pre, _dgrad_pack(conv.weight), cprev, s.hs[k - 1], slope=SLOPE,
-                                                     want_colsum=need_params)
+            if s.bits[k - 1] is not None:
+                d_next, part = ops.conv4x4_dgrad_act(d_pre, _dgrad_pack(conv.weight), cprev, slope=SLOPE,
+                                                     want_colsum=need_params, act_bits=s.bits[k - 1])
                 fused = (d_next, part.sum(0) if part is not None else None)
             else:
                 dh = ops.convT4x4s2_fprop(d_pre, _dgrad_pack(conv.weight), cprev)
diff --git a/thesis-pai-reconstruction_b200/pai_b200/lib.py b/thesis-pai-reconstruction_b200/pai_b200/lib.py
--- a/thesis-pai-reconstruction_b200/pai_b200/lib.py
+++ b/thesis-pai-reconstruction_b200/pai_b200/lib.py
@@ -13,7 +13,7 @@
     "pai_version": [],
     "pai_reserve_sms": [c_int],
     "pai_conv4x4_fprop": [c_void_p, c_int, c_int, c_int, c_int, c_int, c_void_p, c_int, c_int, c_int, c_void_p,
-                          c_int, c_float, c_void_p, c_int, c_int, c_int, c_void_p, c_void_p],
+                          c_int, c_float, c_void_p, c_int, c_int, c_int, c_void_p, c_void_p, c_void_p],
     "pai_convT4x4s2_fprop": [c_void_p, c_int, c_int, c_int, c_int, c_int, c_void_p, c_int, c_int, c_void_p, c_int,
                              c_float, c_void_p, c_int, c_int, c_int, c_void_p, c_void_p],
     "pai_conv4x4_wgrad": [c_void_p, c_int, c_int, c_int, c_int, c_int, c_void_p, c_int, c_int, c_int, c_void_p,
@@ -36,6 +36,7 @@
     "pai_act_bwd": [c_void_p, c_ll, c_int, c_int, c_void_p, c_int, c_int, c_void_p, c_int, c_int, c_float, c_void_p,
                     c_void_p, c_int, c_void_p],
     "pai_colsum": [c_void_p, c_ll, c_int, c_int, c_void_p, c_void_p],
+    "pai_act_sign_bits": [c_void_p, c_ll, c_int, c_int, c_void_p, c_void_p],
     "pai_bn_small_fwd": [c_void_p, c_ll, c_int, c_int, c_void_p, c_void_p, c_float, c_float, c_void_p, c_void_p, c_void_p,
                          c_void_p, c_int, c_int, c_void_p, c_int, c_int, c_float, c_void_p, c_int, c_void_p],
     "pai_bn_small_bwd": [c_void_p, c_ll, c_int, c_int, c_void_p, c_void_p, c_int, c_int, c_void_p, c_int, c_int, c_float,
@@ -110,7 +111,7 @@
                                     c_void_p],
     "pai_check_act_bwd_f32": [c_void_p, c_void_p, c_ll, c_int, c_float, c_void_p, c_void_p],
     "pai_thin_conv4x4s2_fprop": [c_void_p, c_void_p, c_int, c_int, c_int, c_int, c_void_p, c_int, c_void_p, c_void_p, c_int,
-                                 c_int, c_void_p, c_int, c_int, c_float, c_void_p],
+                                 c_int, c_void_p, c_int, c_int, c_float, c_void_p, c_void_p],
     "pai_thin_conv4x4s2_wgrad": [c_void_p, c_int, c_int, c_void_p, c_void_p, c_int, c_int, c_int, c_int, c_void_p, c_void_p],
     "pai_thin_convT4x4s2_plane": [c_void_p, c_int, c_int, c_int, c_int, c_int, c_void_p, c_void_p, c_int, c_void_p, c_void_p],
     "pai_conv4x4_fprop_dual": [c_void_p, c_int, c_int, c_int, c_int, c_int, c_void_p, c_int, c_int, c_int, c_void_p, c_int,
diff --git a/thesis-pai-reconstruction_b200/pai_b200/ops.py b/thesis-pai-reconstruction_b200/pai_b200/ops.py
--- a/thesis-pai-reconstruction_b200/pai_b200/ops.py
+++ b/thesis-pai-reconstruction_b200/pai_b200/ops.py
@@ -152,7 +152,7 @@
 
 
 def conv4x4_fprop(x, w_packed, cout, stride=2, bias=None, act=ACT_NONE, slope=0.2, out=None, out_f32=False,
-                  n_tile=0):
+                  n_tile=0, act_bits=None):
     n, h, w, cin, ld = _nhwc(x)
     cp = w_packed.shape[0]
     ho, wo = (h // 2, w // 2) if stride == 2 else (h - 1, w - 1)
@@ -160,9 +160,30 @@
         out = torch.empty(n, ho, wo, cout, dtype=torch.float32 if out_f32 else torch.bfloat16, device=x.device)
     on, oh, ow, oc, old = _nhwc(out)
     assert (on, oh, ow, oc) == (n, ho, wo, cout)
-    ws = _splitk_ws(n * ho * wo, cout, x.device)
+    ws = None
+    if act_bits is not None:
+        _check_bits(act_bits, out)
+    else:
+        ws = _splitk_ws(n * ho * wo, cout, x.device)
     _igemm_call("pai_conv4x4_fprop", 2.0 * n * ho * wo * cout * 16 * cin, _ptr(x), n, h, w, cin, ld, _ptr(w_packed), cout, cp, stride, _ptr(bias), act,
-             float(slope), _ptr(out), old, int(out.dtype == torch.float32), n_tile, _ptr(ws), _stream())
+             float(slope), _ptr(out), old, int(out.dtype == torch.float32), n_tile, _ptr(ws), _ptr(act_bits), _stream())
+    return out
+
+
+def empty_act_bits(n, h, w, c, device):
+    assert c % 64 == 0
+    return torch.empty(n, h, w, c // 64, dtype=torch.int64, device=device)
+
+
+def _check_bits(bits, act):
+    n, h, w, c = act.shape
+    assert bits.dtype == torch.int64 and bits.is_contiguous() and tuple(bits.shape) == (n, h, w, c // 64) and c % 64 == 0
+
+
+def act_sign_bits(x):
+    n, h, w, c, ld = _nhwc(x)
+    out = empty_act_bits(n, h, w, c, x.device)
+    lib.call("pai_act_sign_bits", _ptr(x), n * h * w, c, ld, _ptr(out), _stream())
     return out
 
 
@@ -217,15 +238,17 @@
     return out, part
 
 
-def conv4x4_dgrad_act(gy, w_packed_dgrad, cin, saved_act, slope=0.2, want_colsum=True):
+def conv4x4_dgrad_act(gy, w_packed_dgrad, cin, saved_act=None, slope=0.2, want_colsum=True, act_bits=None):
     n, h, w, cout, ld = _nhwc(gy)
     cp = w_packed_dgrad.shape[1]
-    sn, sh, sw, sc, sld = _nhwc(saved_act)
-    assert (sn, sh, sw, sc) == (n, 2 * h, 2 * w, cin) and sld == cin
     out = torch.empty(n, 2 * h, 2 * w, cin, dtype=torch.bfloat16, device=gy.device)
+    if act_bits is None:
+        assert tuple(saved_act.shape) == (n, 2 * h, 2 * w, cin)
+        act_bits = act_sign_bits(saved_act)
+    _check_bits(act_bits, out)
     part = zeros_f32(BN_PART_ROWS, 2 * cin, device=gy.device) if want_colsum else None
     _igemm_call("pai_conv4x4_dgrad_act", 2.0 * n * h * w * cin * 16 * cout, _ptr(gy), n, h, w, cout, ld,
-                _ptr(w_packed_dgrad), cin, cp, _ptr(saved_act), float(slope), _ptr(out), cin, 0, _ptr(part), BN_PART_ROWS,
+                _ptr(w_packed_dgrad), cin, cp, _ptr(act_bits), float(slope), _ptr(out), cin, 0, _ptr(part), BN_PART_ROWS,
                 _stream())
     return out, part
 
@@ -463,7 +486,7 @@
     return out
 
 
-def thin_conv_fprop(planes, w_packed, cout, bias, out1, act1=ACT_NONE, out2=None, act2=ACT_NONE, slope=0.2):
+def thin_conv_fprop(planes, w_packed, cout, bias, out1, act1=ACT_NONE, out2=None, act2=ACT_NONE, slope=0.2, act_bits=None):
     p0 = planes[0]
     p1 = planes[1] if len(planes) > 1 else None
     n, ih, iw = p0.shape
@@ -474,9 +497,11 @@
     if out2 is not None:
         assert tuple(out2.shape) == (n, ih // 2, iw // 2, cout)
         ld2 = _nhwc(out2)[4]
+    if act_bits is not None:
+        _check_bits(act_bits, out1)
     _igemm_call("pai_thin_conv4x4s2_fprop", 2.0 * n * (ih // 2) * (iw // 2) * cout * 16 * len(planes), _ptr(p0), _ptr(p1),
                 len(planes), n, ih, iw, _ptr(w_packed), cout, _ptr(bias), _ptr(out1), ld1, act1, _ptr(out2), ld2, act2,
-                float(slope), _stream())
+                float(slope), _ptr(act_bits), _stream())
     return out1
 
 
```

Measured after the change: 9137, median of 6. No clear change (+0.1%).
